# excamera/alfalfa

Measured on AMD Instinct MI355X. Metric: 1080p macroblocks/s decode (bit-exact vs reference), higher is better.
Workload: dtype u8

## Files before the change

### alfalfa_amd/capi.py

```python
import ctypes as C
import os

import numpy as np

from . import build as _build

AA_OK = 0
ERR_NAMES = {-1: "Invalid", -2: "Unsupported", -3: "LogicError", -4: "OutOfRange", -5: "HipError",
             -6: "NoDevice", -7: "BadArgument", -8: "NoMemory"}

AA_MB_HAS_NONZERO, AA_MB_HAS_Y2, AA_MB_INTER, AA_MB_SKIP, AA_MB_LF_SKIP_INNER = 1, 2, 4, 8, 16

MB_INFO_DTYPE = np.dtype([("y_mode", "u1"), ("uv_mode", "u1"), ("ref_frame", "u1"), ("segment_id", "u1"),
                          ("flags", "u1"), ("lf_level", "u1"), ("split_partition", "u1"), ("reserved", "u1"),
                          ("nz_mask", "<u4"), ("coeff_index", "<u4"), ("u", "u1", (64,))])
assert MB_INFO_DTYPE.itemsize == 80


class FrameHeader(C.Structure):
    _fields_ = [(n, C.c_uint8) for n in (
        "key_frame", "show_frame", "loop_filter_level", "sharpness_level", "num_dct_partitions",
        "segmentation_enabled", "filter_adjustments_enabled", "refresh_last", "refresh_golden",
        "refresh_alternate", "copy_buffer_to_golden", "copy_buffer_to_alternate", "sign_bias_golden",
        "sign_bias_alternate", "q_index", "has_intra_mb")] + [
        ("mb_width", C.c_uint16), ("mb_height", C.c_uint16), ("width", C.c_uint16), ("height", C.c_uint16),
        ("quant", (C.c_uint16 * 6) * 4), ("num_macroblocks", C.c_uint32), ("num_coeff_blocks", C.c_uint32),
        ("num_intra_mbs", C.c_uint32), ("compressed_size", C.c_uint32)]

    def as_dict(self):
        d = {n: getattr(self, n) for n, _ in self._fields_ if n != "quant"}
        d["quant"] = [[self.quant[s][k] for k in range(6)] for s in range(4)]
        return d


class FrameIn(C.Structure):
    _fields_ = [("stream", C.c_void_p), ("data", C.c_char_p), ("size", C.c_size_t)]


class KernelStats(C.Structure):
    _fields_ = [("recon_inter_ms", C.c_double), ("recon_intra_ms", C.c_double), ("loopfilter_ms", C.c_double),
                ("recon_inter_launches", C.c_uint64), ("recon_intra_launches", C.c_uint64),
                ("loopfilter_launches", C.c_uint64), ("macroblocks", C.c_uint64),
                ("parse_headers_ms", C.c_double), ("parse_tokens_ms", C.c_double), ("parse_launches", C.c_uint64),
                ("parsed_macroblocks", C.c_uint64), ("recon_split_ms", C.c_double), ("recon_split_launches", C.c_uint64),
                ("pool_waits", C.c_uint64), ("pool_wait_ms", C.c_double), ("parse_wait_ms", C.c_double),
                ("bind_wait_ms", C.c_double), ("alloc_ms", C.c_double), ("slab_mallocs", C.c_uint64),
                ("token_steps", C.c_uint64), ("token_frames", C.c_uint64), ("worker_launches", C.c_uint64), ("worker_wgs", C.c_uint64),
                ("worker_retires", C.c_uint64), ("heap_grows", C.c_uint64), ("heap_mapped_bytes", C.c_uint64), ("nomem_retries", C.c_uint64), ("frames_evicted", C.c_uint64), ("host_routed_frames", C.c_uint64),
                ("row_handoff_stale_polls", C.c_uint64), ("row_handoff_rereads", C.c_uint64), ("packed_frames", C.c_uint64), ("packed_words", C.c_uint64), ("packed_blocks", C.c_uint64),
                ("host_batch_ms", C.c_double), ("host_batch_parse_wall_ms", C.c_double), ("host_batch_parse_cpu_ms", C.c_double), ("host_batch_arena_ms", C.c_double),
                ("pinned_allocs", C.c_uint64)]


class CtxInfo(C.Structure):
    _fields_ = [(n, C.c_uint64) for n in ("memory_limit_bytes", "pool_bytes", "pool_free_bytes", "pool_pending_bytes", "heap_mapped_bytes", "heap_limit_bytes", "heap_used_bytes",
                                          "pinned_host_bytes")] + [
        (n, C.c_uint32) for n in ("heap_is_virtual", "token_lanes_per_workgroup", "token_workgroups_capacity", "token_workgroups_alive",
                                  "token_lane_lds_bytes", "token_workgroup_lds_bytes", "jobs_waiting", "compute_units")] + [
        ("heap_free_chunks", C.c_int32), ("lanes_starved", C.c_uint32), ("token_profile", C.c_uint64 * 8),
        ("packed_coefficients", C.c_uint32), ("lane_per_partition", C.c_uint32), ("clock_mhz", C.c_uint32), ("host_share_ms", C.c_uint32), ("host_rate_kb_per_ms", C.c_uint32), ("reserved1", C.c_uint32), ("stream_concurrency", C.c_uint32), ("streams_needed", C.c_uint32),
        ("host_waited_parse_ms", C.c_uint32), ("host_waited_compute_ms", C.c_uint32)]


AA_RGB_U8_HWC3, AA_RGB_U8_HWC4, AA_RGB_U8_CHW, AA_RGB_F16_CHW, AA_RGB_BF16_CHW, AA_RGB_F32_CHW = range(6)


class RgbTarget(C.Structure):
    _fields_ = [("dst", C.c_void_p), ("row_stride", C.c_int64), ("plane_stride", C.c_int64)]


AA_QUALITY_Y, AA_QUALITY_YUV = 1, 3


class QualityRef(C.Structure):
    _fields_ = [("y", C.c_void_p), ("u", C.c_void_p), ("v", C.c_void_p), ("y_stride", C.c_int64), ("uv_stride", C.c_int64)]


class AlfalfaError(RuntimeError):

    def __init__(self, code, message):
        super().__init__("%s: %s" % (ERR_NAMES.get(code, str(code)), message))
        self.code, self.kind, self.message = code, ERR_NAMES.get(code, str(code)), message


_P = C.c_void_p
_U8P = C.POINTER(C.c_uint8)
SYMBOLS = [
    ("aa_last_error", C.c_char_p, []), ("aa_abi_version", C.c_int, []), ("aa_runtime_prepare", C.c_int, []), ("aa_host_cpus", C.c_int, []), ("aa_device_count", C.c_int, []),
    ("aa_parser_create", C.c_int, [C.c_uint16, C.c_uint16, C.POINTER(_P)]), ("aa_parser_destroy", None, [_P]),
    ("aa_parser_parse", C.c_int, [_P, C.c_char_p, C.c_size_t, C.POINTER(FrameHeader), _P, _P]),
    ("aa_parser_get_probs", C.c_int, [_P, _U8P]), ("aa_parser_set_error_concealment", C.c_int, [_P, C.c_int]),
    ("aa_parse_frame_tag", C.c_int, [C.c_char_p, C.c_size_t, C.c_uint16, C.c_uint16, C.c_int] + [C.POINTER(C.c_int)] * 4),
    ("aa_stream_set_error_concealment", C.c_int, [_P, C.c_int]), ("aa_stream_error_concealment", C.c_int, [_P]),
    ("aa_parser_get_segmentation", C.c_int, [_P, C.POINTER(C.c_int), C.POINTER(C.c_int), C.POINTER(C.c_int8), C.POINTER(C.c_int8), _U8P]),
    ("aa_parser_get_filter_adjustments", C.c_int, [_P, C.POINTER(C.c_int), C.POINTER(C.c_int8), C.POINTER(C.c_int8)]),
    ("aa_parser_serialize_state", C.c_int, [_P, _P, C.c_size_t, _P]), ("aa_parser_deserialize_state", C.c_int, [_P, _P, C.c_size_t]),
    ("aa_stream_serialize", C.c_int, [_P, _P, C.c_size_t, _P]), ("aa_stream_deserialize", C.c_int, [_P, _P, C.c_size_t]),
    ("aa_parser_state_size", C.c_size_t, [_P]), ("aa_parser_export_state", C.c_int, [_P, _P, C.c_size_t]),
    ("aa_parser_import_state", C.c_int, [_P, C.c_char_p, C.c_size_t]),
    ("aa_stream_state_size", C.c_size_t, [_P]), ("aa_stream_export_state", C.c_int, [_P, _P, C.c_size_t]),
    ("aa_stream_import_state", C.c_int, [_P, C.c_char_p, C.c_size_t]),
    ("aa_stream_export_raster", C.c_int, [_P, C.c_int, _P, _P, _P]),
    ("aa_ctx_create", C.c_int, [C.c_int, C.POINTER(_P)]), ("aa_ctx_destroy", None, [_P]), ("aa_ctx_sync", C.c_int, [_P]),
    ("aa_ctx_memory", C.c_int, [_P, C.POINTER(C.c_size_t), C.POINTER(C.c_size_t)]),
    ("aa_ctx_set_memory_limit", C.c_int, [_P, C.c_size_t]), ("aa_ctx_set_packed_coefficients", C.c_int, [_P, C.c_int]), ("aa_ctx_set_host_share_ms", C.c_int, [_P, C.c_double]), ("aa_ctx_set_lane_per_partition", C.c_int, [_P, C.c_int]), ("aa_ctx_get_info", C.c_int, [_P, C.POINTER(CtxInfo)]),
    ("aa_ctx_set_schedule", C.c_int, [_P, C.c_int]), ("aa_ctx_clear_error", C.c_int, [_P]), ("aa_ctx_compute_stream", _P, [_P]), ("aa_ctx_copy_stream", _P, [_P]),
    ("aa_stream_create", C.c_int, [_P, C.c_uint16, C.c_uint16, C.POINTER(_P)]), ("aa_stream_destroy", None, [_P]),
    ("aa_stream_parse", C.c_int, [_P, C.c_char_p, C.c_size_t, C.POINTER(C.c_int), C.POINTER(FrameHeader)]),
    ("aa_stream_append_records", C.c_int, [_P, C.POINTER(FrameHeader), _P, _P, C.POINTER(C.c_int)]),
    ("aa_stream_upload", C.c_int, [_P]), ("aa_stream_release_staging", C.c_int, [_P]),
    ("aa_decode_batch", C.c_int, [_P, C.POINTER(_P), C.c_int, C.POINTER(C.c_int)]),
    ("aa_stream_decode", C.c_int, [_P, C.c_char_p, C.c_size_t, C.POINTER(C.c_int), C.POINTER(C.c_int)]),
    ("aa_submit_frames", C.c_int, [_P, C.POINTER(FrameIn), C.c_int, C.POINTER(C.c_int), C.c_int]),
    ("aa_submit_frames_ex", C.c_int, [_P, C.POINTER(FrameIn), C.c_int, C.POINTER(C.c_int), C.c_int, C.c_uint]),
    ("aa_launch_tokens", C.c_int, [_P, C.c_int, C.POINTER(C.c_int)]),
    ("aa_ssim_host", C.c_int, [C.c_char_p, C.c_char_p, C.c_int, C.c_int, C.POINTER(C.c_double)]),
    ("aa_stream_lf_search", C.c_int, [_P, C.c_char_p, C.c_size_t, C.c_void_p, C.c_int, C.c_int, C.POINTER(C.c_int), C.POINTER(C.c_double),
                                      C.POINTER(C.c_double), C.c_void_p]),
    ("aa_stream_frame_header", C.c_int, [_P, C.c_int, C.POINTER(FrameHeader)]),
    ("aa_stream_read_records", C.c_int, [_P, C.c_int, _P, _P, C.c_size_t]),
    ("aa_stream_frame_count", C.c_int, [_P]), ("aa_stream_release_before", C.c_int, [_P, C.c_int]),
    ("aa_stream_rewind", C.c_int, [_P]), ("aa_stream_rewind_to", C.c_int, [_P, C.c_int]),
    ("aa_stream_download", C.c_int, [_P, C.c_int, _P, _P, _P]),
    ("aa_pinned_alloc", C.c_int, [_P, C.c_size_t, C.POINTER(_P)]), ("aa_pinned_free", None, [_P]),
    ("aa_stream_download_async", C.c_int, [_P, C.c_int, _P, _P, _P]), ("aa_stream_download_wait", C.c_int, [_P]),
    ("aa_download_batch_async", C.c_int, [_P, C.POINTER(_P), C.c_int, C.POINTER(C.c_int), _P, C.c_size_t]), ("aa_ctx_download_wait", C.c_int, [_P]), ("aa_ctx_download_wait_until", C.c_int, [_P, C.c_int]),
    ("aa_stream_raster_device", C.c_int, [_P, C.c_int, C.POINTER(_P), C.POINTER(_P), C.POINTER(_P)]),
    ("aa_render_rgb_async", C.c_int, [_P, C.POINTER(_P), C.c_int, C.POINTER(C.c_int), C.c_int, C.POINTER(RgbTarget),
                                      C.POINTER(C.c_double), C.POINTER(C.c_double), _P]),
    ("aa_quality_batch_async", C.c_int, [_P, C.POINTER(_P), C.c_int, C.POINTER(C.c_int), C.POINTER(QualityRef), C.c_int, _P, _P, _P]),
    ("aa_stream_references", C.c_int, [_P, C.POINTER(C.c_int), C.POINTER(C.c_int), C.POINTER(C.c_int)]),
    ("aa_stream_reference_slots", C.c_int, [_P, C.POINTER(C.c_int)]),
    ("aa_stream_import_reference", C.c_int, [_P, _P, _P, _P]),
    ("aa_stream_import_reference_host", C.c_int, [_P, _P, _P, _P]),
# ... 54 lines not shown
```

### alfalfa_amd/csrc/device_types.h

```cpp
#pragma once
#include <stdint.h>

#include "../../include/alfalfa_amd.h"

struct aa_dev_frame {
  uint8_t * cur[3];
  const uint8_t * ref[4][3];
  const aa_mb_info * mbs;
  const int16_t * coeffs;
  const unsigned long long * intra_rows;
  uint16_t quant[4][6];
  uint16_t mbw, mbh;
  uint8_t key_frame;
  uint8_t loop_filter_level;
  uint8_t sharpness;
  uint8_t has_intra;
  uint32_t packed;
};

struct aa_raster_binding {
  aa_dev_frame * job;
  uint8_t * cur[3];
  const uint8_t * ref[3][3];
};

struct aa_gather_job {
  const uint8_t * src;
  size_t bytes;
};

struct aa_rgb_job {
  const uint8_t * plane[3];
  uint8_t * dst;
  int64_t row_stride, plane_stride;
  uint32_t stride_y, stride_c;
  uint32_t width, height;
  uint32_t groups;
  uint32_t pad;
};

#define AA_QUALITY_STRIP_ROWS 8
#define AA_QUALITY_CHUNK_WINDOWS 480
struct aa_quality_job {
  const uint8_t * a, * b;
  int64_t stride_a, stride_b;
  uint32_t w4, h4;
  uint32_t groups;
  uint32_t strips, chunks;
  uint32_t pad;
  uint64_t out_off;
};

#define AA_MAX_XCD 16

#define AA_SYNC_WS_DUMP 140
#define AA_SYNC_WS_RESCUES 132
struct aa_sync_ws {
  int error;
  int where[3];
  int dump[AA_SYNC_WS_DUMP];
  int ticket[AA_MAX_XCD];
  int progress[1];
};
#define AA_SYNC_WS_ZERO_FROM ( 16 + 4 * AA_SYNC_WS_DUMP )

#define AA_MAX_BATCH 480

struct aa_frame_list {
  const aa_dev_frame * f[AA_MAX_BATCH];
};

struct aa_seg_stream { uint8_t * map; uint32_t first, count; };

#define AA_MAX_WORKER_GRIDS 16
struct aa_tok_mirror {
  uint32_t seq;
  uint32_t q_head, q_publish, q_reserve;
  int32_t pool_avail;
  uint32_t pool_starving;
  uint32_t exited[AA_MAX_WORKER_GRIDS];
  unsigned long long prof[8];
};

namespace aa {
struct ParseJob;
struct TokQueue; struct CoeffPool; struct Heap;
int launch_parse_mb_headers( const ParseJob * jobs, const uint32_t * order, int n, void * stream );
int launch_segment_fixup( const ParseJob * jobs, const aa_seg_stream * streams, int n_streams, const uint32_t * order, void * stream );
void token_worker_shape( uint32_t lane_bytes, int n_cus, int * lanes_out, uint32_t * lds_out, int * wgs_per_cu_out );
int launch_token_workers( TokQueue * q, unsigned long long * slots, const Heap & heap, uint32_t * exited, const uint32_t * retire, uint32_t gen, uint32_t spread,
                          unsigned long long * prof, unsigned long long linger_ticks, int wgs, int lanes, uint32_t lane_bytes, uint32_t lds, bool packed, uint32_t mp_hint, void * stream,
                          uint32_t * cu_slots = nullptr, uint32_t cu_cap = 0 );
#define AA_CU_SLOTS ( 16 * 256 )
int launch_enqueue_jobs( TokQueue * q, unsigned long long * slots, const ParseJob * jobs, const uint32_t * order, int n, void * stream );
int launch_pool_push_range( const Heap & heap, uint32_t first, uint32_t count, void * stream );
int launch_pool_free_lists( const Heap & heap, const uint32_t * const * lists, int n, void * stream );
int launch_mirror_counters( const TokQueue * q, const CoeffPool * pool, const uint32_t * exited, int n_grids, const unsigned long long * prof, aa_tok_mirror * out, uint32_t seq, void * stream );
int launch_recon_inter4( const aa_frame_list & list, int n, unsigned max_mbs, void * stream );
int launch_recon_inter( const aa_frame_list & list, int n, unsigned max_mbs, bool split_only, void * stream );
int launch_recon_intra_diagonal( const aa_frame_list & list, int n, int diagonal, int row_lo, int rows, void * stream );
int launch_loopfilter_diagonal( const aa_frame_list & list, int n, int diagonal, int row_lo, int rows, void * stream );
int launch_recon_intra4( const aa_frame_list & list, int n_groups, int mbh_max, aa_sync_ws * ws, int n_xcd, void * stream );
int launch_loopfilter_rows4( const aa_frame_list & list, int n_groups, int mbh_max, int mbw_max, aa_sync_ws * ws, uint8_t * boundary, int n_xcd, void * stream );
int launch_probe_xcds( int * out16, int blocks, void * stream );
int launch_probe_concurrency( uint32_t * counter, uint32_t * seen, uint32_t n, unsigned long long timeout_ticks, int slot, void * stream );
int launch_bind_rasters( const aa_raster_binding * b, int n, void * stream );
int launch_gather_rasters( const aa_gather_job * jobs, int n, uint8_t * staging, size_t stride, size_t max_bytes, void * stream );
int launch_render_rgb( const aa_rgb_job * jobs, int n, int format, const uint32_t * table, uint32_t max_threads, void * stream );
int launch_lf_relevel( const aa_mb_info * src, aa_mb_info * dst, unsigned nmb, uint32_t levels, void * stream );
int launch_ssim_windows( const uint8_t * a, const uint8_t * b, int width, int height, float * out, void * stream );
int launch_quality( const aa_quality_job * jobs, int n_planes, uint32_t max_blocks, float * group_values, double * ssim, unsigned long long * sse, void * stream );
}
```

### alfalfa_amd/csrc/parse_kernels.hip

```cpp
#include <hip/hip_runtime.h>

#include <algorithm>

#include "device_types.h"
#include "tok_fsm.hh"
#include "coeff_pack.hh"

#ifndef AA_WORKER_PRIO
#define AA_WORKER_PRIO 3
#endif

namespace {

using aa::ParseJob;

__global__ __launch_bounds__( 64 ) void k_parse_mb_headers( const ParseJob * jobs, const uint32_t * order, int n, int lanes )
{
  __builtin_amdgcn_s_setprio( 2 );

  __shared__ aa::HeaderTables s_tables;
  __shared__ aa::HeaderParams s_params[16];
  const int lane = threadIdx.x;
  for ( uint32_t k = lane; k < sizeof( aa::HeaderTables ) / 4; k += 64 ) reinterpret_cast<uint32_t *>( &s_tables )[k] = reinterpret_cast<const uint32_t *>( &aa::kHeaderTables )[k];
  const int slot = blockIdx.x * lanes + lane;
  const bool mine = lane < lanes && lane < 16 && slot < n;
  const ParseJob * Jp = mine ? &jobs[order[slot]] : nullptr;
  if ( Jp ) {
    const uint32_t * src = reinterpret_cast<const uint32_t *>( static_cast<const aa::HeaderParams *>( &Jp->fp ) );
    for ( uint32_t k = 0; k < sizeof( aa::HeaderParams ) / 4; k++ ) reinterpret_cast<uint32_t *>( &s_params[lane] )[k] = src[k];
  }
  __syncthreads();
  if ( !Jp ) return;
  const ParseJob & J = *Jp;
  if ( J.nmb == 0 ) return;
  const aa::HeaderParams & fp = s_params[lane];
  const aa::HeaderTables & T = s_tables;
  aa::BoolReader32 bd;
  aa::BoolState st; st.bitpos = fp.bd_bitpos; st.range = fp.bd_range; st.active = fp.bd_active;
  bd.resume( J.data + fp.first_off, fp.first_size, st );
  const unsigned mbw = fp.mbw, mbh = fp.mbh;
  const unsigned words_per_row = ( mbw + 63 ) / 64;
  uint32_t intra = 0, split = 0;
  unsigned mi = 0;
  const uint32_t mp_stride = J.mp_stride, mp_base = J.flags_padded, nparts = fp.nparts;
  for ( unsigned row = 0; row < mbh; row++ ) {
    unsigned long long word = 0;
    const uint32_t mp_row = mp_stride ? mp_base + ( row % nparts ) * mp_stride + ( row / nparts ) * mbw : 0u;
    for ( unsigned col = 0; col < mbw; col++, mi++ ) {
      const uint8_t flags = aa::parse_mb_header( bd, fp, T, J.mbs, mi, col, row, static_cast<uint8_t *>( nullptr ) );
      J.mbflags[mi] = flags;
      if ( mp_stride ) J.mbflags[mp_row + col] = flags;
      if ( !( flags & AA_MB_INTER ) ) { intra++; word |= 1ull << ( col & 63 ); }
      else if ( J.mbs[mi].y_mode == aa::SPLITMV ) split = 1;
      if ( ( col & 63 ) == 63 || col + 1 == mbw ) { J.intra_rows[row * words_per_row + ( col >> 6 )] = word; word = 0; }
    }
  }
  J.summary->num_intra_mbs = intra;
  J.summary->has_split = split;
}

__global__ __launch_bounds__( 256 ) void k_segment_fixup( const ParseJob * jobs, const aa_seg_stream * streams, const uint32_t * order )
{
  const aa_seg_stream s = streams[blockIdx.x];
  for ( uint32_t k = 0; k < s.count; k++ ) {
    const uint32_t o = order[s.first + k];
    const ParseJob & J = jobs[o & 0x7FFFFFFFu];
    if ( !J.fp.seg_enabled || J.nmb == 0 ) continue;
    if ( o >> 31 ) {
      for ( uint32_t mi = threadIdx.x; mi < J.nmb; mi += blockDim.x ) s.map[mi] = 3;
      __syncthreads();
    }
    for ( uint32_t mi = threadIdx.x; mi < J.nmb; mi += blockDim.x ) aa::segment_fixup( J.fp, J.mbs[mi], s.map[mi] );
    __syncthreads();
  }
}

struct WorkerArgs {
  aa::TokQueue * q;
  unsigned long long * slots;
  aa::Heap heap;
  uint32_t * exited;
  const uint32_t * retire;
  uint32_t gen;
  uint32_t spread;
  unsigned long long * prof;
  unsigned long long linger_ticks;
  int lanes;
  uint32_t lane_bytes;
  uint32_t mp_hint;
  uint32_t * cu_slots;
  uint32_t cu_cap;
  int16_t * sink;
};

__device__ inline uint32_t queue_take( aa::TokQueue * q, uint32_t want, uint32_t spread, uint32_t * base )
{
  uint32_t h = AA_AT_LOAD( &q->head );
  for ( uint32_t tries = 0; ; tries++ ) {
    const uint32_t avail = AA_AT_LOAD( &q->publish ) - h;
    if ( static_cast<int32_t>( avail ) <= 0 ) return 0;
    const uint32_t share = ( avail + spread - 1u ) / spread;
    const uint32_t n = want < share ? want : share;
    uint32_t expect = h;
    if ( __hip_atomic_compare_exchange_strong( &q->head, &expect, h + n, __ATOMIC_RELAXED, __ATOMIC_RELAXED, __HIP_MEMORY_SCOPE_AGENT ) ) { *base = h; return n; }
    h = expect;
    const uint32_t r = ( blockIdx.x * 2654435761u + tries * 40503u ) >> 27;
    for ( uint32_t k = 0; k <= ( r & ( tries < 4 ? 3u : tries < 8 ? 15u : 31u ) ); k++ ) __builtin_amdgcn_s_sleep( 16 );
    if ( tries > 2048 ) h = AA_AT_LOAD( &q->head );
  }
}

__device__ inline int nth_set_bit( unsigned long long mask, uint32_t n )
{
  for ( uint32_t k = 0; k < n; k++ ) mask &= mask - 1ull;
  return __ffsll( static_cast<long long>( mask ) ) - 1;
}

template <bool PK, bool MP>
__global__ __launch_bounds__( 64 ) void k_token_workers( const WorkerArgs a )
{
  extern __shared__ __attribute__( ( aligned( 16 ) ) ) uint8_t smem[];
  const int lane = threadIdx.x;
#if AA_WORKER_PRIO
  __builtin_amdgcn_s_setprio( AA_WORKER_PRIO );
#endif
  uint32_t cu_slot = 0;
  if ( a.cu_slots ) {
    const uint32_t hw = __builtin_amdgcn_s_getreg( 4 | ( 8 << 6 ) | ( 7 << 11 ) ), xcc = __builtin_amdgcn_s_getreg( 20 | ( 0 << 6 ) | ( 3 << 11 ) );
    cu_slot = ( ( xcc & 15u ) << 8 ) | ( hw & 255u );
    uint32_t before = 0;
    if ( lane == 0 ) before = AA_AT_ADD( &a.cu_slots[cu_slot], 1u );
    before = __shfl( before, 0 );
    if ( before >= a.cu_cap ) {
      if ( lane == 0 ) { AA_AT_ADD( &a.cu_slots[cu_slot], 0xFFFFFFFFu ); AA_AT_ADD( &a.cu_slots[AA_CU_SLOTS - 1], 1u ); AA_AT_ADD( a.exited, 1u ); }
      return;
    }
  }
  for ( uint32_t k = lane; k < aa::tok::kTablesBytes / 4; k += 64 ) reinterpret_cast<uint32_t *>( smem )[k] = aa::tok::table_word( k );
  __syncthreads();
  aa::tok::Lane L;
  aa::tok::Frame F {};
// ... 79 lines not shown
      }
      backoff = 0;
      continue;
    }
    idle_since = 0;
    const unsigned long long t_b = profiling ? wall_clock64() : 0ull;
    if ( active ) aa::tok::top_up<MP>( L, smem, F );
    const unsigned long long t_c = profiling ? wall_clock64() : 0ull;
    aa::tok::run_period<PK, MP>( L, smem, F, a.heap, profiling, pp );
    if ( profiling ) {
      const unsigned long long t_d = wall_clock64();
      p_look += t_b - t_a; p_topup += t_c - t_b; p_period += t_d - t_c;
      p_lanes += static_cast<unsigned long long>( __popcll( __ballot( active ) ) ); p_periods++;
      if ( ( p_periods & 1023ull ) == 0 ) {
        if ( lane == 0 ) prof_flush();
        pp = { 0, 0, 0 }; p_look = p_topup = p_period = p_lanes = p_periods = 0;
      }
    }
  }
  if ( lane == 0 ) {
    if ( profiling ) prof_flush();
    if ( a.cu_slots ) AA_AT_ADD( &a.cu_slots[cu_slot], 0xFFFFFFFFu );
    AA_AT_ADD( a.exited, 1u );
  }
}

__global__ __launch_bounds__( 64 ) void k_enqueue_jobs( aa::TokQueue * q, unsigned long long * slots, const ParseJob * jobs, const uint32_t * order, int n )
{
  __shared__ uint32_t s_base;
  if ( threadIdx.x == 0 ) s_base = AA_AT_ADD( &q->reserve, static_cast<uint32_t>( n ) );
  __syncthreads();
  const uint32_t base = s_base, mask = q->mask;
  for ( int i = threadIdx.x; i < n; i += 64 ) AA_AT_STORE( &slots[( base + i ) & mask], reinterpret_cast<unsigned long long>( &jobs[order[i]] ) );
  __syncthreads();
  if ( threadIdx.x == 0 ) {
    __builtin_amdgcn_fence( __ATOMIC_RELEASE, "agent" );
    asm volatile( "s_waitcnt vmcnt(0)" ::: "memory" );
    while ( AA_AT_LOAD( &q->publish ) != base ) __builtin_amdgcn_s_sleep( 8 );
    AA_AT_STORE( &q->publish, base + static_cast<uint32_t>( n ) );
  }
}

__device__ inline void pool_push_wave( const aa::Heap & H, const AA_GLOBAL uint32_t * ids, uint32_t first, uint32_t n_mine )
{
  __shared__ uint32_t s_off[65];
  __shared__ uint32_t s_pbase;
  s_off[threadIdx.x + 1] = n_mine;
  __syncthreads();
  if ( threadIdx.x == 0 ) {
    s_off[0] = 0;
    for ( int i = 1; i <= 64; i++ ) s_off[i] += s_off[i - 1];
    s_pbase = s_off[64] ? AA_AT_ADD( &H.pool->reserve, s_off[64] ) : 0u;
  }
  __syncthreads();
  const uint32_t b = s_pbase + s_off[threadIdx.x], mask = H.pool->mask, total = s_off[64];
  for ( uint32_t i = 0; i < n_mine; i++ ) AA_AT_STORE( &H.ring[( b + i ) & mask], ids ? ids[i] : first + i );
  __syncthreads();
  if ( threadIdx.x == 0 && total ) {
    __builtin_amdgcn_fence( __ATOMIC_RELEASE, "agent" );
    asm volatile( "s_waitcnt vmcnt(0)" ::: "memory" );
    while ( AA_AT_LOAD( &H.pool->publish ) != s_pbase ) __builtin_amdgcn_s_sleep( 8 );
    AA_AT_STORE( &H.pool->publish, s_pbase + total );
    AA_AT_ADD_REL( &H.pool->avail, static_cast<int32_t>( total ) );
  }
}
__global__ __launch_bounds__( 64 ) void k_pool_push_range( aa::Heap heap, uint32_t first, uint32_t count )
{
  const uint32_t per = ( count + 63u ) / 64u, lo = threadIdx.x * per;
  const uint32_t mine = lo >= count ? 0u : ( count - lo < per ? count - lo : per );
  pool_push_wave( heap, nullptr, first + lo, mine );
}
struct FreeLists { const uint32_t * l[AA_MAX_BATCH]; };
__global__ __launch_bounds__( 64 ) void k_pool_free_lists( aa::Heap heap, const FreeLists lists, int n )
{
  const int i = blockIdx.x * 64 + threadIdx.x;
  const AA_GLOBAL uint32_t * l = ( i < n && lists.l[i] ) ? (const AA_GLOBAL uint32_t *) lists.l[i] : nullptr;
  pool_push_wave( heap, l ? l + 1 : nullptr, 0, l ? l[0] : 0u );
}
__global__ void k_mirror_counters( const aa::TokQueue * q, const aa::CoeffPool * pool, const uint32_t * exited, int n_grids, const unsigned long long * prof, aa_tok_mirror * out, uint32_t seq )
{
  if ( threadIdx.x || blockIdx.x ) return;
  if ( prof ) for ( int k = 0; k < 8; k++ ) out->prof[k] = AA_AT_LOAD( &prof[k] );
  out->q_head = AA_AT_LOAD( &q->head ); out->q_publish = AA_AT_LOAD( &q->publish ); out->q_reserve = AA_AT_LOAD( &q->reserve );
  if ( pool ) { out->pool_avail = AA_AT_LOAD( &pool->avail ); out->pool_starving = AA_AT_LOAD( &pool->starving ); }
  for ( int g = 0; g < n_grids; g++ ) out->exited[g] = AA_AT_LOAD( &exited[g] );
  __builtin_amdgcn_fence( __ATOMIC_RELEASE, "" );
  asm volatile( "s_waitcnt vmcnt(0)" ::: "memory" );
  __hip_atomic_store( &out->seq, seq, __ATOMIC_RELAXED, __HIP_MEMORY_SCOPE_SYSTEM );
}

}

namespace aa {

static int parse_lanes_env()
{
  static const int lanes = [] {
    const char * e = getenv( "ALFALFA_AMD_PARSE_LANES" );
    const int v = e ? atoi( e ) : 0;
    return v < 0 ? 0 : ( v > 64 ? 64 : v );
  }();
  return lanes;
}
static int header_lanes() { const int v = parse_lanes_env(); return v ? std::min( v, 16 ) : 16; }

constexpr uint32_t kLdsPerCu = 160u * 1024u, kLdsGranule = 512u;
static uint32_t env_u32( const char * name, uint32_t dflt ) { const char * e = getenv( name ); return e ? static_cast<uint32_t>( atoi( e ) ) : dflt; }
static const uint32_t kWgsPerCu = std::max( 1u, std::min( 16u, env_u32( "ALFALFA_AMD_WGS_PER_CU", 3u ) ) );
static const uint32_t kMaxLanes = std::max( 1u, std::min( 64u, env_u32( "ALFALFA_AMD_MAX_LANES", 30u ) ) );
struct TokenShape { int lanes; uint32_t lds; int per_cu; };
static TokenShape token_launch_shape( uint32_t lane_bytes )
{
  for ( uint32_t n = kWgsPerCu; n >= 1; n-- ) {
    const uint32_t request = std::min( 65536u, ( kLdsPerCu / ( n + 1 ) / kLdsGranule + 1 ) * kLdsGranule );
    if ( request < tok::kTablesBytes + lane_bytes || request * n > kLdsPerCu ) continue;
    const int lanes = static_cast<int>( std::min<uint32_t>( kMaxLanes, ( request - tok::kTablesBytes ) / lane_bytes ) );
    return { lanes, request, static_cast<int>( n ) };
  }
  return { 0, 0, 0 };
}

int launch_parse_mb_headers( const ParseJob * jobs, const uint32_t * order, int n, void * stream )
{
  const int lanes = header_lanes();
  hipLaunchKernelGGL( k_parse_mb_headers, dim3( ( n + lanes - 1 ) / lanes ), dim3( 64 ), 0, static_cast<hipStream_t>( stream ), jobs, order, n, lanes );
  return static_cast<int>( hipGetLastError() );
}

int launch_segment_fixup( const ParseJob * jobs, const aa_seg_stream * streams, int n_streams, const uint32_t * order, void * stream )
{
  hipLaunchKernelGGL( k_segment_fixup, dim3( n_streams ), dim3( 256 ), 0, static_cast<hipStream_t>( stream ), jobs, streams, order );
  return static_cast<int>( hipGetLastError() );
}

void token_worker_shape( uint32_t lane_bytes, int n_cus, int * lanes_out, uint32_t * lds_out, int * wgs_per_cu_out )
{
  int lanes = parse_lanes_env();
  uint32_t lds = 0;
  if ( lanes ) {
    if ( static_cast<uint32_t>( lanes ) * lane_bytes + tok::kTablesBytes > 65536u ) lanes = static_cast<int>( ( 65536u - tok::kTablesBytes ) / lane_bytes );
    lds = static_cast<uint32_t>( lanes ) * lane_bytes + tok::kTablesBytes;
  } else {
    const TokenShape sh = token_launch_shape( lane_bytes );
    lanes = sh.lanes; lds = sh.lds;
  }
  (void) n_cus;
  static const bool lds_exact = env_u32( "ALFALFA_AMD_LDS_EXACT", 1u ) != 0u;
  static const uint32_t wgs_cap = env_u32( "ALFALFA_AMD_WGS_CAP_PER_CU", lds_exact && !parse_lanes_env() ? kWgsPerCu : 0u );
  if ( lds_exact && lanes > 0 ) lds = ( ( tok::kTablesBytes + static_cast<uint32_t>( lanes ) * lane_bytes + kLdsGranule - 1u ) / kLdsGranule ) * kLdsGranule;
  *lanes_out = lanes; *lds_out = lds;
  int per_cu = lds ? static_cast<int>( kLdsPerCu / lds ) : 0;
  if ( wgs_cap && per_cu > static_cast<int>( wgs_cap ) ) per_cu = static_cast<int>( wgs_cap );
  *wgs_per_cu_out = per_cu;
}

int launch_token_workers( TokQueue * q, unsigned long long * slots, const Heap & heap, uint32_t * exited, const uint32_t * retire, uint32_t gen, uint32_t spread,
                          unsigned long long * prof, unsigned long long linger_ticks, int wgs, int lanes, uint32_t lane_bytes, uint32_t lds, bool packed, uint32_t mp_hint, void * stream,
                          uint32_t * cu_slots, uint32_t cu_cap )
{
  if ( lanes < 1 || wgs < 1 ) return static_cast<int>( hipErrorInvalidValue );
  WorkerArgs a;
  a.q = q; a.slots = slots; a.heap = heap; a.exited = exited; a.retire = retire; a.gen = gen; a.spread = spread ? spread : 1u; a.prof = prof; a.linger_ticks = linger_ticks; a.lanes = lanes; a.lane_bytes = lane_bytes;
  a.mp_hint = mp_hint ? mp_hint : 1u;
  a.cu_slots = cu_cap ? cu_slots : nullptr; a.cu_cap = cu_cap;
  a.sink = reinterpret_cast<int16_t *>( cu_slots + AA_CU_SLOTS / 2 );
  if ( mp_hint ) {
    if ( packed ) hipLaunchKernelGGL( ( k_token_workers<true, true> ), dim3( wgs ), dim3( 64 ), lds, static_cast<hipStream_t>( stream ), a );
    else hipLaunchKernelGGL( ( k_token_workers<false, true> ), dim3( wgs ), dim3( 64 ), lds, static_cast<hipStream_t>( stream ), a );
  } else {
    if ( packed ) hipLaunchKernelGGL( ( k_token_workers<true, false> ), dim3( wgs ), dim3( 64 ), lds, static_cast<hipStream_t>( stream ), a );
    else hipLaunchKernelGGL( ( k_token_workers<false, false> ), dim3( wgs ), dim3( 64 ), lds, static_cast<hipStream_t>( stream ), a );
  }
  return static_cast<int>( hipGetLastError() );
}

int launch_enqueue_jobs( TokQueue * q, unsigned long long * slots, const ParseJob * jobs, const uint32_t * order, int n, void * stream )
{
  hipLaunchKernelGGL( k_enqueue_jobs, dim3( 1 ), dim3( 64 ), 0, static_cast<hipStream_t>( stream ), q, slots, jobs, order, n );
  return static_cast<int>( hipGetLastError() );
}

int launch_pool_push_range( const Heap & heap, uint32_t first, uint32_t count, void * stream )
{
  hipLaunchKernelGGL( k_pool_push_range, dim3( 1 ), dim3( 64 ), 0, static_cast<hipStream_t>( stream ), heap, first, count );
  return static_cast<int>( hipGetLastError() );
}

int launch_pool_free_lists( const Heap & heap, const uint32_t * const * lists, int n, void * stream )
{
  for ( int base = 0; base < n; base += AA_MAX_BATCH ) {
    FreeLists fl;
    const int cnt = std::min( AA_MAX_BATCH, n - base );
    for ( int i = 0; i < AA_MAX_BATCH; i++ ) fl.l[i] = i < cnt ? lists[base + i] : nullptr;
    hipLaunchKernelGGL( k_pool_free_lists, dim3( ( cnt + 63 ) / 64 ), dim3( 64 ), 0, static_cast<hipStream_t>( stream ), heap, fl, cnt );
    if ( hipError_t e = hipGetLastError() ) return static_cast<int>( e );
  }
  return 0;
}

int launch_mirror_counters( const TokQueue * q, const CoeffPool * pool, const uint32_t * exited, int n_grids, const unsigned long long * prof, aa_tok_mirror * out, uint32_t seq, void * stream )
{
  hipLaunchKernelGGL( k_mirror_counters, dim3( 1 ), dim3( 64 ), 0, static_cast<hipStream_t>( stream ), q, pool, exited, n_grids, prof, out, seq );
  return static_cast<int>( hipGetLastError() );
}

}
```

### alfalfa_amd/csrc/runtime_ctx.inc

```

extern "C" {

const char * aa_last_error( void ) { return g_last_error.c_str(); }
int aa_host_cpus( void ) { return effective_cpus(); }
int aa_runtime_prepare( void )
{
  const bool was_set = std::getenv( "GPU_MAX_HW_QUEUES" ) != nullptr;
  setenv( "GPU_MAX_HW_QUEUES", "16", 0 );
  return was_set ? 1 : 0;
}
int aa_abi_version( void ) { return AA_ABI_VERSION; }
int aa_device_count( void ) { int n = 0; if ( hipGetDeviceCount( &n ) != hipSuccess ) return 0; return n; }

void aa_raster_geometry( uint16_t width, uint16_t height, uint32_t * pw, uint32_t * ph )
{
  if ( pw ) *pw = 16u * ( ( width + 15u ) / 16u );
  if ( ph ) *ph = 16u * ( ( height + 15u ) / 16u );
}

aa_status aa_parser_create( uint16_t width, uint16_t height, aa_parser ** out )
{
  if ( !out || !width || !height ) return fail( AA_ERR_ARGUMENT, "aa_parser_create: bad argument" );
  *out = new ( std::nothrow ) aa_parser( width, height );
  return *out ? AA_OK : fail( AA_ERR_ARGUMENT, "out of memory" );
// ... 265 lines not shown
    out->memory_limit_bytes = ctx->pool_soft_limit; out->pool_bytes = ctx->pool_bytes; out->pinned_host_bytes = ctx->pinned_bytes;
    for ( auto & kv : ctx->dev_free ) out->pool_free_bytes += kv.first * kv.second.size();
    for ( auto & pf : ctx->pending_free ) out->pool_pending_bytes += pf.bytes;
    if ( ctx->cur_slab ) out->pool_free_bytes += kSlabBytes - ctx->slab_used;
    out->pool_free_bytes += ctx->compute_free_bytes;
    for ( auto & h : ctx->compute_hold ) out->pool_pending_bytes += h.second;
  }
  out->heap_mapped_bytes = T.heap_mapped; out->heap_limit_bytes = T.heap_va;
  out->heap_used_bytes = static_cast<uint64_t>( std::max<int64_t>( 0, T.chunks_committed ) ) * kChunkBytesHeap;
  out->heap_is_virtual = T.vmm ? 1u : 0u;
  out->packed_coefficients = T.packed ? 1u : 0u;
  out->lane_per_partition = T.lane_per_partition ? 1u : 0u;
  out->token_lanes_per_workgroup = static_cast<uint32_t>( T.lanes ); out->token_workgroups_capacity = static_cast<uint32_t>( T.cap_wgs );
  out->token_lane_lds_bytes = T.lane_bytes; out->token_workgroup_lds_bytes = T.lds;
  out->compute_units = static_cast<uint32_t>( T.n_cus );
  out->host_share_ms = static_cast<uint32_t>( ctx->host_share_ms + 0.5 );
  out->host_rate_kb_per_ms = ctx->host_lanes.parse_us.load() ? static_cast<uint32_t>( host_lanes_rate( ctx ) / 1e3 + 0.5 ) : 0u;
  out->stream_concurrency = ctx->stream_concurrency; out->streams_needed = ctx->streams_needed;
  out->host_waited_parse_ms = static_cast<uint32_t>( ctx->stats.parse_wait_ms ); out->host_waited_compute_ms = static_cast<uint32_t>( ctx->stats.bind_wait_ms );
  if ( !ctx->clock_mhz ) { int khz = 0; if ( hipDeviceGetAttribute( &khz, hipDeviceAttributeClockRate, ctx->device ) == hipSuccess ) ctx->clock_mhz = static_cast<uint32_t>( khz / 1000 ); else (void) hipGetLastError(); }
  out->clock_mhz = ctx->clock_mhz;
  if ( T.ready ) {
    if ( aa_status st = tok_peek_mirror( ctx ) ) return st;
    out->heap_free_chunks = T.mirror_host->pool_avail; out->lanes_starved = T.mirror_host->pool_starving;
    for ( int k = 0; k < 8; k++ ) out->token_profile[k] = T.mirror_host->prof[k];
    uint32_t alive = 0;
    for ( int g = 0; g < aa_ctx::Tok::kSlots; g++ ) alive += T.slot[g].launched - T.mirror_host->exited[g];
    out->token_workgroups_alive = alive;
    const int32_t waiting = static_cast<int32_t>( static_cast<uint32_t>( T.jobs_enqueued ) - T.mirror_host->q_head );
    out->jobs_waiting = waiting > 0 ? static_cast<uint32_t>( waiting ) : 0u;
  }
  return AA_OK;
}
aa_status aa_ctx_set_lane_per_partition( aa_ctx * ctx, int on )
{
  if ( !ctx ) return fail( AA_ERR_ARGUMENT, "null context" );
  if ( ctx->tok.ready && ctx->tok.lane_per_partition != ( on != 0 ) ) return fail( AA_ERR_LOGIC, "aa_ctx_set_lane_per_partition: frames have been submitted to this context already" );
  ctx->tok.lane_per_partition = on != 0;
  return AA_OK;
}
aa_status aa_ctx_set_host_share_ms( aa_ctx * ctx, double ms )
{
  if ( !ctx || !( ms >= 0 ) ) return fail( AA_ERR_ARGUMENT, "aa_ctx_set_host_share_ms: bad argument" );
  ctx->host_share_ms = ms;
  return AA_OK;
}
aa_status aa_ctx_set_packed_coefficients( aa_ctx * ctx, int on )
{
  if ( !ctx ) return fail( AA_ERR_ARGUMENT, "null context" );
  if ( ctx->tok.ready && ctx->tok.packed != ( on != 0 ) ) return fail( AA_ERR_LOGIC, "aa_ctx_set_packed_coefficients: frames have been submitted to this context already" );
  ctx->tok.packed = on != 0;
  return AA_OK;
}
aa_status aa_ctx_clear_error( aa_ctx * ctx )
{
  if ( !ctx ) return fail( AA_ERR_ARGUMENT, "null ctx" );
  if ( aa_status st = set_device( ctx ) ) return st;
  HIP_TRY( hipStreamSynchronize( ctx->compute ) );
  if ( ctx->ws ) { HIP_TRY( hipMemsetAsync( ctx->ws, 0, AA_SYNC_WS_ZERO_FROM, ctx->compute ) ); HIP_TRY( hipStreamSynchronize( ctx->compute ) ); }
  return AA_OK;
}
aa_status aa_ctx_set_schedule( aa_ctx * ctx, int schedule )
{
  if ( !ctx || ( schedule != AA_SCHEDULE_ROWS && schedule != AA_SCHEDULE_DIAGONAL ) ) return fail( AA_ERR_ARGUMENT, "aa_ctx_set_schedule: bad argument" );
  ctx->schedule = schedule;
  return AA_OK;
}
void * aa_ctx_compute_stream( aa_ctx * ctx ) { return ctx ? ctx->compute : nullptr; }
void * aa_ctx_copy_stream( aa_ctx * ctx ) { return ctx ? ctx->copy : nullptr; }
aa_status aa_ctx_profile( aa_ctx * ctx, int enable )
{
  if ( !ctx ) return fail( AA_ERR_ARGUMENT, "null ctx" );
  if ( !enable ) { (void) hipStreamSynchronize( ctx->compute ); for ( auto ps : ctx->parse_streams ) (void) hipStreamSynchronize( ps ); drain_profile( ctx ); }
  ctx->profile = enable != 0;
  return AA_OK;
}
aa_status aa_ctx_kernel_stats( aa_ctx * ctx, aa_kernel_stats * out, int reset )
{
  if ( !ctx || !out ) return fail( AA_ERR_ARGUMENT, "null argument" );
  HIP_TRY( hipStreamSynchronize( ctx->compute ) );
  for ( auto ps : ctx->parse_streams ) HIP_TRY( hipStreamSynchronize( ps ) );
  drain_profile( ctx );
  ctx->stats.heap_mapped_bytes = ctx->tok.heap_mapped;
  if ( ctx->ws ) {
    int rescued[6] = {};
    HIP_TRY( hipMemcpy( rescued, &ctx->ws->dump[AA_SYNC_WS_RESCUES], sizeof rescued, hipMemcpyDeviceToHost ) );
    ctx->stats.row_handoff_rereads = static_cast<uint64_t>( rescued[0] );
    ctx->stats.row_handoff_stale_polls = static_cast<uint64_t>( rescued[3] );
    ctx->row_handoff_by_kernel[0] = rescued[4]; ctx->row_handoff_by_kernel[1] = rescued[5];
    if ( const char * e = std::getenv( "ALFALFA_AMD_HANDOFF_REPORT" ) ) if ( atoi( e ) )
      std::fprintf( stderr, "alfalfa_amd: row hand-off waits ended by the second look: %d (k_recon_intra4 %d, k_loopfilter_rows4 %d); system-scope load saw it %d, L2 read-modify-write %d; poll repeated still stale %d\n",
                    rescued[0], rescued[4], rescued[5], rescued[1], rescued[2], rescued[3] );
  }
  const uint64_t lanes_us = ctx->host_lanes.parse_us.load();
  ctx->stats.host_batch_parse_cpu_ms = static_cast<double>( lanes_us - ctx->host_lanes.parse_us_mark ) / 1e3;
  *out = ctx->stats;
  if ( reset ) { ctx->stats = aa_kernel_stats {}; ctx->host_lanes.parse_us_mark = lanes_us; }
  return AA_OK;
}

aa_status aa_stream_create( aa_ctx * ctx, uint16_t width, uint16_t height, aa_stream ** out )
{
  if ( !ctx || !out || !width || !height ) return fail( AA_ERR_ARGUMENT, "aa_stream_create: bad argument" );
  if ( aa_status st = set_device( ctx ) ) return st;
  std::unique_ptr<aa_stream> s( new aa_stream( ctx, width, height ) );
  aa_raster_geometry( width, height, &s->pw, &s->ph );
  s->plane_bytes[0] = size_t( s->pw ) * s->ph;
  s->plane_bytes[1] = s->plane_bytes[2] = size_t( s->pw / 2 ) * ( s->ph / 2 );
  s->slot_bytes = align_up( s->plane_bytes[0] + 2 * s->plane_bytes[1] );
  uint8_t * blank = nullptr;
  {
    std::lock_guard<std::mutex> g( ctx->blank_mu );
    auto it = ctx->blank.find( s->slot_bytes );
    if ( it != ctx->blank.end() ) blank = it->second;
    else {
      if ( aa_status st = dev_alloc( ctx, s->slot_bytes, &blank ) ) return st;
      hipError_t e = hipMemsetAsync( blank, 0, s->slot_bytes, ctx->compute );
      if ( e == hipSuccess ) e = hipStreamSynchronize( ctx->compute );
      if ( e != hipSuccess ) { dev_free( ctx, blank, s->slot_bytes ); return hip_fail( e, "hipMemsetAsync (blank reference raster)" ); }
      ctx->blank[s->slot_bytes] = blank;
    }
  }
  Slot sl; sl.dev = blank; sl.shared = true;
  s->slots.push_back( sl );
  const int slot = 0;
  for ( int i = 0; i < 3; i++ ) { s->cur_ref_slot[i] = -1; s->cur_ref_frame[i] = -1; }
  for ( int i = 0; i < 3; i++ ) set_ref( s.get(), i, slot, -1 );
  ctx->refs++;
  *out = s.release();
  return AA_OK;
}
void aa_stream_destroy( aa_stream * s )
{
  if ( !s ) return;
  aa_ctx * ctx = s->ctx;
  (void) hipSetDevice( ctx->device );
  bool staged = false;
  for ( auto & c : s->chunks ) if ( c.host && c.uploaded ) staged = true;
  if ( staged ) (void) hipStreamSynchronize( ctx->copy );
  for ( auto & f : s->frames ) if ( f.batch && f.batch->hdr_done && !f.enqueued && !f.records_released ) (void) hipEventSynchronize( f.batch->hdr_done );
  for ( auto & f : s->frames ) release_records( s, f, true );
  for ( auto & c : s->chunks ) {
    if ( c.host ) { std::lock_guard<std::mutex> g( ctx->pool_mu ); ctx->pinned_pool.emplace_back( c.host, c.pinned_bytes ); c.host = nullptr; }
    if ( c.dev ) { dev_free( ctx, c.dev, c.dev_bytes, true ); c.dev = nullptr; }
  }
  for ( auto & sl : s->slots ) if ( sl.dev && !sl.shared ) dev_free_compute( ctx, sl.dev, s->slot_bytes );
  dev_free( ctx, s->dev_segmap, size_t( s->parser.mb_width() ) * s->parser.mb_height(), true );
  delete s;
  if ( --ctx->refs == 0 ) ctx_free( ctx );
}

}
```

### alfalfa_amd/csrc/runtime_decode.inc

```
extern "C" {

static aa_status resolve_summary( aa_stream * s, FrameRec & r )
{
  if ( !r.summary_pending ) return AA_OK;
  aa_ctx * ctx = s->ctx;
  auto & T = ctx->tok;
  Batch * b = r.batch;
  if ( !b || !r.summary ) return fail( AA_ERR_LOGIC, "frame records were released before the frame was decoded" );
  if ( b->tokens_pending ) if ( aa_status st = launch_tokens_of( ctx, b ) ) return st;
  volatile aa::FrameSummary * sum = r.summary;
  for ( int attempt = 0; ; attempt++ ) {
    if ( aa_status st = tok_wait_done( ctx, sum ) ) return st;
    if ( sum->status != aa::TOK_NO_MEMORY ) break;
    ctx->stats.nomem_retries++;
    const uint32_t worst = aa::chunk_list_entries( r.hdr.num_macroblocks, T.lane_per_partition ? 8u : 1u );
    {
      std::lock_guard<std::mutex> g( ctx->pool_mu );
      if ( !r.chunks_returned ) { T.pending_lists.push_back( r.chunk_list ); r.chunks_returned = true; T.chunks_committed -= r.est_chunks; r.est_chunks = 0; }
      flush_chunk_frees( ctx );
      if ( !T.pending_lists.empty() ) return fail( AA_ERR_HIP, "k_pool_free_lists could not be launched" );
    }
    HIP_TRY( hipStreamSynchronize( ctx->compute ) );
    if ( aa_status st = tok_grow_heap( ctx, T.heap_mapped + static_cast<size_t>( worst ) * kChunkBytesHeap ) ) return st;
    if ( aa_status st = tok_refresh_mirror( ctx ) ) return st;
    if ( T.mirror_host->pool_avail < static_cast<int32_t>( worst ) ) {
      if ( aa_status st = tok_quiesce( ctx ) ) return st;
      if ( aa_status st = tok_refresh_mirror( ctx ) ) return st;
    }
    if ( T.mirror_host->pool_avail < static_cast<int32_t>( worst ) ) {
      int32_t have = T.mirror_host->pool_avail;
      std::lock_guard<std::mutex> g( ctx->pool_mu );
      for ( auto bi = T.batches.rbegin(); bi != T.batches.rend() && have < static_cast<int32_t>( worst ); ++bi ) {
        Batch * vb = *bi;
        volatile aa::FrameSummary * sums = reinterpret_cast<volatile aa::FrameSummary *>( vb->host + vb->summaries_off );
        for ( int i = vb->n - 1; i >= 0 && have < static_cast<int32_t>( worst ); i-- ) {
          if ( !vb->items[i].live ) continue;
          aa_stream * vs = vb->items[i].s;
          FrameRec & v = vs->frames[vb->items[i].frame];
          if ( &v == &r || vb->items[i].on_host || !v.enqueued || v.records_released || v.chunks_returned || !sums[i].done || vb->items[i].frame < vs->next_submit ) continue;
          T.pending_lists.push_back( v.chunk_list );
          have += static_cast<int32_t>( sums[i].num_chunks );
          v.chunks_returned = true; v.summary_pending = true;
          T.chunks_committed -= v.est_chunks; v.est_chunks = 0;
          sums[i].status = aa::TOK_NO_MEMORY;
          ctx->stats.frames_evicted++;
        }
      }
      flush_chunk_frees( ctx );
      if ( !T.pending_lists.empty() ) return fail( AA_ERR_HIP, "k_pool_free_lists could not be launched" );
    }
    HIP_TRY( hipStreamSynchronize( ctx->compute ) );
    if ( aa_status st = tok_refresh_mirror( ctx ) ) return st;
    if ( attempt >= 8 || T.mirror_host->pool_avail < static_cast<int32_t>( worst ) )
      return fail( AA_ERR_NO_MEMORY, "device parser: the coefficient heap is exhausted (" + std::to_string( T.heap_mapped >> 20 ) + " MiB mapped, "
                                     + std::to_string( T.mirror_host->pool_avail ) + " chunks free, this frame may need " + std::to_string( worst )
                                     + "): release decoded frames (aa_stream_release_before) or raise the limit (aa_ctx_set_memory_limit); the call can be repeated" );
    sum->status = 0; sum->done = 0; sum->num_chunks = 0;
    r.chunks_returned = false;
    r.est_chunks = worst; T.chunks_committed += worst;
    __atomic_thread_fence( __ATOMIC_SEQ_CST );
    if ( int e = aa::launch_enqueue_jobs( T.q, T.slots, r.parse_job, T.one_dev, 1, T.util ) ) return hip_fail( static_cast<hipError_t>( e ), "k_enqueue_jobs" );
    T.jobs_enqueued += 1;
    if ( std::find( T.inflight.begin(), T.inflight.end(), b ) == T.inflight.end() ) T.inflight.push_back( b );
    if ( aa_status st = tok_service( ctx ) ) return st;
  }
  if ( sum->status == aa::TOK_HOST_FAILED ) return fail( AA_ERR_HIP, "host lane: the frame's records could not be placed in device memory" );
  if ( sum->status == aa::TOK_STEP_BOUND ) return fail( AA_ERR_HIP, "device parser: a token lane exceeded the step bound of its frame size (records are not valid)" );
  r.hdr.num_coeff_blocks = sum->num_coeff_blocks;
  r.hdr.num_intra_mbs = sum->num_intra_mbs;
  r.hdr.has_intra_mb = sum->num_intra_mbs != 0;
  r.has_split = sum->has_split != 0;
  r.intra_diagonals.assign( r.hdr.mb_width + 2 * ( r.hdr.mb_height - 1 ), r.hdr.has_intra_mb ? 1 : 0 );
  T.chunks_committed += static_cast<int64_t>( sum->num_chunks ) - static_cast<int64_t>( r.est_chunks );
  r.est_chunks = sum->num_chunks;
  if ( r.hdr.compressed_size ) T.blocks_per_byte += 0.05 * ( static_cast<double>( sum->num_coeff_blocks ) / r.hdr.compressed_size - T.blocks_per_byte );
  if ( r.hdr.compressed_size && r.packed_pos ) T.words_per_byte += 0.05 * ( static_cast<double>( sum->packed_words ) / r.hdr.compressed_size - T.words_per_byte );
  if ( r.packed_pos ) { ctx->stats.packed_frames++; ctx->stats.packed_words += sum->packed_words; ctx->stats.packed_blocks += sum->num_coeff_blocks; }
  ctx->stats.token_steps += sum->steps; ctx->stats.token_frames++;
  r.summary_pending = false;
  return AA_OK;
}

aa_status aa_stream_frame_header( aa_stream * s, int fi, aa_frame_header * out )
{
  if ( !s || !out || fi < 0 || fi >= static_cast<int>( s->frames.size() ) ) return fail( AA_ERR_ARGUMENT, "aa_stream_frame_header: bad argument" );
  if ( aa_status st = set_device( s->ctx ) ) return st;
  if ( aa_status st = resolve_summary( s, s->frames[fi] ) ) return st;
  *out = s->frames[fi].hdr;
  return AA_OK;
}

aa_status aa_stream_read_records( aa_stream * s, int fi, aa_mb_info * mb_out, int16_t * coeff_out, size_t coeff_capacity_blocks )
{
  if ( !s || fi < 0 || fi >= static_cast<int>( s->frames.size() ) ) return fail( AA_ERR_ARGUMENT, "aa_stream_read_records: bad argument" );
  if ( aa_status st = set_device( s->ctx ) ) return st;
  FrameRec & r = s->frames[fi];
  if ( r.records_released ) return fail( AA_ERR_LOGIC, "aa_stream_read_records: frame records were released" );
  if ( aa_status st = resolve_summary( s, r ) ) return st;
  if ( aa_status st = aa_stream_upload( s ) ) return st;
  HIP_TRY( hipStreamSynchronize( s->ctx->copy ) );
  aa_dev_frame job;
  HIP_TRY( hipMemcpy( &job, r.dev_job, sizeof job, hipMemcpyDeviceToHost ) );
  if ( coeff_out && coeff_capacity_blocks < r.hdr.num_coeff_blocks ) return fail( AA_ERR_ARGUMENT, "aa_stream_read_records: coefficient buffer too small" );
  if ( !r.chunk_list ) {
    if ( mb_out ) HIP_TRY( hipMemcpy( mb_out, job.mbs, size_t( r.hdr.num_macroblocks ) * sizeof( aa_mb_info ), hipMemcpyDeviceToHost ) );
    if ( coeff_out ) HIP_TRY( hipMemcpy( coeff_out, job.coeffs, size_t( r.hdr.num_coeff_blocks ) * 32, hipMemcpyDeviceToHost ) );
    return AA_OK;
  }
  std::vector<aa_mb_info> mbs( r.hdr.num_macroblocks );
  HIP_TRY( hipMemcpy( mbs.data(), job.mbs, mbs.size() * sizeof( aa_mb_info ), hipMemcpyDeviceToHost ) );
  std::vector<uint32_t> list( size_t( r.est_chunks ) + 1 );
  HIP_TRY( hipMemcpy( list.data(), r.chunk_list, list.size() * sizeof( uint32_t ), hipMemcpyDeviceToHost ) );
  if ( list[0] != r.est_chunks ) return fail( AA_ERR_LOGIC, "aa_stream_read_records: chunk list disagrees with the parse summary" );
  if ( r.packed_pos ) {
    std::vector<uint32_t> pos( r.hdr.num_macroblocks );
    HIP_TRY( hipMemcpy( pos.data(), r.packed_pos, pos.size() * sizeof( uint32_t ), hipMemcpyDeviceToHost ) );
    std::vector<std::vector<int16_t>> words( list[0] );
    if ( coeff_out )
      for ( uint32_t k = 0; k < list[0]; k++ ) {
        words[k].resize( aa::kChunkWords );
        HIP_TRY( hipMemcpy( words[k].data(), s->ctx->tok.heap + size_t( list[1 + k] ) * kChunkBytesHeap, kChunkBytesHeap, hipMemcpyDeviceToHost ) );
      }
    uint32_t running = 0;
    for ( size_t mi = 0; mi < mbs.size(); mi++ ) {
      aa_mb_info & mb = mbs[mi];
      const uint32_t nblk = aa::pack::blocks_of( mb.nz_mask );
      if ( nblk && coeff_out ) {
        const uint32_t ord = pos[mi] >> 15, off = pos[mi] & ( aa::kChunkWords - 1u );
        if ( ord >= list[0] || running + nblk > r.hdr.num_coeff_blocks )
          return fail( AA_ERR_LOGIC, "aa_stream_read_records: a macroblock's coefficients lie outside the frame's chunks" );
        const int16_t * w = words[ord].data() + off, * end = words[ord].data() + aa::kChunkWords;
        if ( w + aa::pack::kMaskSlots > end ) return fail( AA_ERR_LOGIC, "aa_stream_read_records: packed coefficients run past their chunk" );
        uint32_t values = 0;
        for ( uint32_t b = 0; b < 25; b++ ) if ( ( mb.nz_mask >> b ) & 1u ) values += aa::pack::popc( static_cast<uint16_t>( w[b] ) );
        if ( w + aa::pack::kMaskSlots + values > end ) return fail( AA_ERR_LOGIC, "aa_stream_read_records: packed coefficients run past their chunk" );
        if ( ( static_cast<unsigned long long>( mb.reserved ) << 32 | mb.coeff_index ) != static_cast<unsigned long long>( list[1 + ord] ) * aa::kChunkWords + off )
          return fail( AA_ERR_LOGIC, "aa_stream_read_records: a macroblock's word offset disagrees with its place in the frame's chunks" );
        aa::pack::expand_macroblock( w, mb.nz_mask, coeff_out + size_t( running ) * 16 );
      }
      mb.coeff_index = running; mb.reserved = 0;
      running += nblk;
    }
    if ( running != r.hdr.num_coeff_blocks ) return fail( AA_ERR_LOGIC, "aa_stream_read_records: non-zero masks disagree with the parse summary" );
    if ( mb_out ) std::memcpy( mb_out, mbs.data(), mbs.size() * sizeof( aa_mb_info ) );
    return AA_OK;
  }
  std::map<uint32_t, std::vector<uint8_t>> chunk;
  if ( coeff_out )
    for ( uint32_t k = 0; k < list[0]; k++ ) {
// ... 263 lines not shown
```

### alfalfa_amd/csrc/runtime_records.inc

```

static uint8_t * slot_plane( aa_stream * s, int slot, int plane )
{
  uint8_t * p = s->slots[slot].dev;
  if ( plane >= 1 ) p += s->plane_bytes[0];
  if ( plane >= 2 ) p += s->plane_bytes[1];
  return p;
}

namespace {

void release_records( aa_stream * s, FrameRec & f, bool deferred )
{
  if ( f.records_released ) return;
  aa_ctx * ctx = s->ctx;
  bool parsed = false;
  if ( f.enqueued && f.summary ) parsed = tok_wait_done( ctx, f.summary ) == AA_OK;
  if ( !parsed && f.enqueued && f.summary && f.batch && f.batch_item >= 0 && f.batch_item < static_cast<int>( f.batch->items.size() ) && f.batch->items[f.batch_item].on_host ) {
    while ( !summary_done( f.summary ) ) usleep( 200 );
  }
  f.records_released = true;
  if ( f.rec_block ) {
    const bool has_chunks = parsed && f.chunk_list && !f.chunks_returned;
    if ( has_chunks ) { std::lock_guard<std::mutex> g( ctx->pool_mu ); ctx->tok.pending_lists.push_back( f.chunk_list ); ctx->open_epoch_used = true; f.chunks_returned = true; }
    if ( !f.rec_in_arena ) dev_free( ctx, f.rec_block, f.rec_bytes, deferred || has_chunks );
    f.rec_block = nullptr; f.chunk_list = nullptr; f.packed_pos = nullptr;
    ctx->tok.chunks_committed -= f.est_chunks; f.est_chunks = 0;
  }
  if ( Batch * b = f.batch ) {
    if ( f.batch_item >= 0 && f.batch_item < static_cast<int>( b->items.size() ) ) {
      Batch::Item & bi = b->items[f.batch_item];
      if ( bi.host_dense ) { dev_free( ctx, bi.host_dense, bi.host_dense_bytes, true ); bi.host_dense = nullptr; }
    }
    bool last;
    { std::lock_guard<std::mutex> g( ctx->pool_mu ); last = --b->live == 0; }
    if ( f.batch_item >= 0 && f.batch_item < static_cast<int>( b->items.size() ) ) b->items[f.batch_item].live = false;
    if ( last ) {
      if ( b->tokens_pending ) ctx->deferred.erase( std::remove( ctx->deferred.begin(), ctx->deferred.end(), b ), ctx->deferred.end() );
      ctx->tok.inflight.erase( std::remove( ctx->tok.inflight.begin(), ctx->tok.inflight.end(), b ), ctx->tok.inflight.end() );
      ctx->tok.batches.erase( std::remove( ctx->tok.batches.begin(), ctx->tok.batches.end(), b ), ctx->tok.batches.end() );
      if ( b->hdr_done ) { (void) hipEventSynchronize( b->hdr_done ); (void) hipEventDestroy( b->hdr_done ); }
      { std::lock_guard<std::mutex> g( ctx->pool_mu ); ctx->pinned_pool.emplace_back( b->host, b->host_bytes ); }
      dev_free( ctx, b->dev, b->dev_bytes, true );
      delete b;
    }
    f.batch = nullptr; f.summary = nullptr; f.parse_job = nullptr;
  }
  if ( f.chunk >= 0 && f.chunk < static_cast<int>( s->chunks.size() ) ) {
    Chunk & c = s->chunks[f.chunk];
    const bool is_tail = f.chunk + 1 == static_cast<int>( s->chunks.size() ) && c.host != nullptr;
    if ( --c.live_frames == 0 && !is_tail && c.dev ) {
      if ( c.host ) { std::lock_guard<std::mutex> g( ctx->pool_mu ); ctx->pinned_pool.emplace_back( c.host, c.pinned_bytes ); c.host = nullptr; }
      dev_free( ctx, c.dev, c.dev_bytes, deferred ); c.dev = nullptr;
    }
  }
  f.host_job = nullptr; f.dev_job = nullptr;
}

uint8_t * pinned_get( aa_ctx * ctx, size_t bytes, size_t * got )
{
  {
    std::lock_guard<std::mutex> g( ctx->pool_mu );
    auto & pool = ctx->pinned_pool;
    for ( size_t i = 0; i < pool.size(); i++ )
      if ( pool[i].second >= bytes && pool[i].second <= bytes + bytes / 2 ) {
        uint8_t * p = pool[i].first; *got = pool[i].second;
        pool[i] = pool.back(); pool.pop_back();
        return p;
      }
  }
  uint8_t * p = nullptr;
  if ( hipHostMalloc( reinterpret_cast<void **>( &p ), bytes, hipHostMallocDefault ) != hipSuccess ) return nullptr;
  *got = bytes;
  { std::lock_guard<std::mutex> g( ctx->pool_mu ); ctx->pinned_bytes += bytes; ctx->stats.pinned_allocs++; }
  return p;
}

void fill_job( const FrameRec & rec, aa_dev_frame * job )
{
  const aa_frame_header & h = rec.hdr;
  std::memset( job, 0, sizeof *job );
  std::memcpy( job->quant, h.quant, sizeof job->quant );
  job->mbw = h.mb_width; job->mbh = h.mb_height;
  job->key_frame = h.key_frame; job->loop_filter_level = h.loop_filter_level;
  job->sharpness = h.sharpness_level; job->has_intra = h.has_intra_mb;
}

aa_status bind_frame( aa_stream * s, int fi, aa_raster_binding * out )
{
  FrameRec & rec = s->frames[fi];
  const aa_frame_header & h = rec.hdr;
  int out_slot;
  if ( aa_status st = alloc_slot( s, &out_slot ) ) return st;
  retain( s, out_slot );
  rec.out_slot = out_slot;
  out->job = const_cast<aa_dev_frame *>( rec.dev_job );
  for ( int p = 0; p < 3; p++ ) out->cur[p] = slot_plane( s, out_slot, p );
  for ( int r = 0; r < 3; r++ ) for ( int p = 0; p < 3; p++ ) out->ref[r][p] = slot_plane( s, s->cur_ref_slot[r], p );
  enum { LAST = 0, GOLDEN = 1, ALT = 2 };
  if ( h.key_frame ) { for ( int i = 0; i < 3; i++ ) set_ref( s, i, out_slot, fi ); }
  else {
    if ( h.copy_buffer_to_alternate == 1 ) set_ref( s, ALT, s->cur_ref_slot[LAST], s->cur_ref_frame[LAST] );
    else if ( h.copy_buffer_to_alternate == 2 ) set_ref( s, ALT, s->cur_ref_slot[GOLDEN], s->cur_ref_frame[GOLDEN] );
    if ( h.copy_buffer_to_golden == 1 ) set_ref( s, GOLDEN, s->cur_ref_slot[LAST], s->cur_ref_frame[LAST] );
    else if ( h.copy_buffer_to_golden == 2 ) set_ref( s, GOLDEN, s->cur_ref_slot[ALT], s->cur_ref_frame[ALT] );
    if ( h.refresh_golden ) set_ref( s, GOLDEN, out_slot, fi );
    if ( h.refresh_alternate ) set_ref( s, ALT, out_slot, fi );
    if ( h.refresh_last ) set_ref( s, LAST, out_slot, fi );
  }
  for ( int i = 0; i < 3; i++ ) rec.ref_after[i] = s->cur_ref_frame[i];
  rec.placed = true;
  if ( !rec.handle_held ) release( s, out_slot );
  return AA_OK;
}

aa_status bind_batch( aa_ctx * ctx, aa_stream * const * streams, int n, const int * frame_index )
{
  int need = 0;
  for ( int i = 0; i < n; i++ ) if ( !streams[i]->frames[frame_index[i]].placed ) need++;
  if ( !need ) return AA_OK;
  aa_ctx::BindBuf & bb = ctx->bind_bufs[ctx->next_bind_buf];
  ctx->next_bind_buf = ( ctx->next_bind_buf + 1 ) % aa_ctx::kBindBufs;
  if ( bb.busy ) {
    const auto t0 = std::chrono::steady_clock::now();
// ... 37 lines not shown
```

### alfalfa_amd/csrc/runtime_submit.inc

```
namespace {
template <class Fill>
aa_status append_host_frame( aa_stream * s, int * frame_index, aa_frame_header * hdr_out, Fill && fill )
{
  if ( aa_status st = set_device( s->ctx ) ) return st;
  const size_t nmb = size_t( s->parser.mb_width() ) * s->parser.mb_height();
  const size_t job_bytes = align_up( sizeof( aa_dev_frame ) );
  const size_t mb_bytes = align_up( nmb * sizeof( aa_mb_info ) );
  const size_t words_per_row = ( s->parser.mb_width() + 63 ) / 64;
  const size_t rows_bytes = align_up( words_per_row * s->parser.mb_height() * sizeof( unsigned long long ) );
  const size_t worst = job_bytes + mb_bytes + rows_bytes + align_up( nmb * 25 * 32 );
  Chunk * c;
  if ( aa_status st = reserve( s, worst, &c ) ) return st;
  const size_t off = c->used;
  aa_dev_frame * job = reinterpret_cast<aa_dev_frame *>( c->host + off );
  aa_mb_info * mbs = reinterpret_cast<aa_mb_info *>( c->host + off + job_bytes );
  unsigned long long * intra_rows = reinterpret_cast<unsigned long long *>( c->host + off + job_bytes + mb_bytes );
  int16_t * coeffs = reinterpret_cast<int16_t *>( c->host + off + job_bytes + mb_bytes + rows_bytes );

  FrameRec rec;
  try { fill( rec.hdr, mbs, coeffs ); }
  catch ( const aa::ParseError & e ) { return fail( e.code, e.message ); }
  const aa_frame_header & h = rec.hdr;
  c->used = off + job_bytes + mb_bytes + rows_bytes + align_up( size_t( h.num_coeff_blocks ) * 32 );

// ... 55 lines not shown
  }
  return append_host_frame( s, frame_index, nullptr, [&]( aa_frame_header & h, aa_mb_info * mbs, int16_t * coeffs ) {
    h = *hdr;
    h.num_intra_mbs = intra; h.has_intra_mb = intra != 0;
    std::memcpy( mbs, mbs_in, nmb * sizeof( aa_mb_info ) );
    if ( hdr->num_coeff_blocks ) std::memcpy( coeffs, coeffs_in, size_t( hdr->num_coeff_blocks ) * 32 );
  } );
}

aa_status aa_stream_upload( aa_stream * s )
{
  if ( !s ) return fail( AA_ERR_ARGUMENT, "null stream" );
  if ( aa_status st = set_device( s->ctx ) ) return st;
  bool any = false;
  for ( auto & c : s->chunks ) {
    if ( c.host && c.uploaded < c.used ) {
      HIP_TRY( hipMemcpyAsync( c.dev + c.uploaded, c.host + c.uploaded, c.used - c.uploaded, hipMemcpyHostToDevice, s->ctx->copy ) );
      c.uploaded = c.used; any = true;
    }
  }
  if ( any ) {
    HIP_TRY( hipEventRecord( s->ctx->upload_done, s->ctx->copy ) );
    HIP_TRY( hipStreamWaitEvent( s->ctx->compute, s->ctx->upload_done, 0 ) );
  }
  return AA_OK;
}

aa_status aa_stream_release_staging( aa_stream * s )
{
  if ( !s ) return fail( AA_ERR_ARGUMENT, "null stream" );
  if ( aa_status st = set_device( s->ctx ) ) return st;
  if ( aa_status st = aa_stream_upload( s ) ) return st;
  HIP_TRY( hipStreamSynchronize( s->ctx->copy ) );
  for ( auto & c : s->chunks ) {
    if ( !c.host ) continue;
    { std::lock_guard<std::mutex> g( s->ctx->pool_mu ); s->ctx->pinned_pool.emplace_back( c.host, c.pinned_bytes ); }
    c.host = nullptr;
    c.capacity = c.used;
  }
  for ( auto & f : s->frames ) f.host_job = nullptr;
  return AA_OK;
}


namespace {
struct SubmitItem {
  aa_stream * s; const uint8_t * data; size_t size;
  size_t data_off;
  size_t rec_off = 0;
  aa_status status = AA_OK; std::string error;
  int frame_index = -1;
  bool seg_enabled = false, seg_reset = false;
  bool on_host = false;
};

aa_status submit_one( Batch * b, SubmitItem & it, int item, aa::ParseJob * jobs_host, aa_dev_frame * dframes_host, bool want_host_lane )
{
  aa_stream * s = it.s;
  aa_ctx * ctx = s->ctx;
  aa::ParseJob & J = jobs_host[item];
  FrameRec rec;
  try { s->parser.parse_header( it.data, it.size, rec.hdr, J.fp ); }
  catch ( const aa::ParseError & e ) { it.error = e.message; return e.code; }
  it.seg_enabled = J.fp.seg_enabled; it.seg_reset = s->parser.segment_map_reset();
  std::memcpy( b->host + it.data_off, it.data, it.size );

  const uint32_t nmb = uint32_t( J.fp.mbw ) * J.fp.mbh;
  const size_t mb_bytes = align_up( size_t( nmb ) * sizeof( aa_mb_info ) );
  const size_t words_per_row = ( J.fp.mbw + 63 ) / 64;
  const size_t rows_bytes = align_up( words_per_row * J.fp.mbh * sizeof( unsigned long long ) );
  const uint32_t flags_padded = ( nmb + 15u ) & ~15u;
  const bool mp = ctx->tok.lane_per_partition && J.fp.nparts > 1;
  const uint32_t mp_stride = mp ? aa::mp_flag_stride( J.fp.mbw, J.fp.mbh, J.fp.nparts ) : 0u;
  const size_t flags_bytes = align_up( size_t( flags_padded ) + size_t( J.fp.nparts ) * mp_stride );
  const size_t list_bytes = align_up( size_t( aa::chunk_list_entries( nmb, mp ? J.fp.nparts : 1u ) ) * sizeof( uint32_t ) );

  const size_t pos_bytes = ctx->tok.packed ? align_up( size_t( nmb ) * sizeof( uint32_t ) ) : 0;
  rec.rec_bytes = mb_bytes + rows_bytes + flags_bytes + list_bytes + pos_bytes;
  rec.rec_block = b->dev + it.rec_off; rec.rec_in_arena = true;
  uint8_t * blk = rec.rec_block;

  J.data = b->dev + it.data_off;
  J.size = static_cast<uint32_t>( it.size ); J.data_padded = ( J.size + 15u ) & ~15u;
  J.nmb = nmb; J.flags_padded = flags_padded; J.mp_stride = mp_stride; J.mp_pad = 0;
  J.mbs = reinterpret_cast<aa_mb_info *>( blk );
  J.intra_rows = reinterpret_cast<unsigned long long *>( blk + mb_bytes );
  J.mbflags = blk + mb_bytes + rows_bytes;
  J.chunk_list = reinterpret_cast<uint32_t *>( blk + mb_bytes + rows_bytes + flags_bytes );
  J.packed_pos = pos_bytes ? reinterpret_cast<uint32_t *>( blk + mb_bytes + rows_bytes + flags_bytes + list_bytes ) : nullptr;
  rec.packed_pos = J.packed_pos; rec.dev_mbs = J.mbs;
  J.summary = reinterpret_cast<aa::FrameSummary *>( b->host_dev + b->summaries_off ) + item;
  rec.chunk_list = J.chunk_list;
  rec.summary = reinterpret_cast<volatile aa::FrameSummary *>( b->host + b->summaries_off ) + item;
  rec.parse_job = reinterpret_cast<const aa::ParseJob *>( b->dev ) + item;

  aa_dev_frame * job = &dframes_host[item];
  rec.hdr.has_intra_mb = 1;
  fill_job( rec, job );
  job->mbs = J.mbs; job->intra_rows = J.intra_rows;
  job->coeffs = reinterpret_cast<const int16_t *>( ctx->tok.heap );
  job->packed = ctx->tok.packed ? 1u : 0u;
  rec.host_job = job;
  rec.dev_job = reinterpret_cast<const aa_dev_frame *>( b->dev + ( reinterpret_cast<uint8_t *>( job ) - b->host ) );
  rec.batch = b; rec.batch_item = item; rec.summary_pending = true;
  if ( want_host_lane && !J.fp.seg_enabled ) {
    it.on_host = true;
    job->packed = 0;
    rec.packed_pos = nullptr; rec.chunk_list = nullptr;
    rec.enqueued = true;
  }
  it.frame_index = static_cast<int>( s->frames.size() );
  s->frames.push_back( std::move( rec ) );
  return AA_OK;
}
}

namespace {
aa_status launch_tokens_of( aa_ctx * ctx, Batch * b )
{
  if ( !b->tokens_pending ) return AA_OK;
  auto & T = ctx->tok;
  aa::ParseJob * jobs_host = reinterpret_cast<aa::ParseJob *>( b->host );
  if ( static_cast<uint32_t>( T.jobs_enqueued ) - T.mirror_host->q_head + static_cast<uint32_t>( b->n ) + 4096u > T.q_slots ) {
    if ( aa_status st = tok_refresh_mirror( ctx ) ) return st;
    if ( static_cast<uint32_t>( T.jobs_enqueued ) - T.mirror_host->q_head + static_cast<uint32_t>( b->n ) + 4096u > T.q_slots )
      if ( aa_status st = tok_quiesce( ctx ) ) return st;
  }
  b->tokens_pending = false;
  ctx->deferred.erase( std::remove( ctx->deferred.begin(), ctx->deferred.end(), b ), ctx->deferred.end() );
  bool dropped = false;
  tok_prune_inflight( ctx );
  for ( int i = 0; i < b->n; i++ ) {
    Batch::Item & it = b->items[i];
    if ( !it.live ) { if ( jobs_host[i].nmb ) { jobs_host[i].nmb = 0; dropped = true; } continue; }
    FrameRec & r = it.s->frames[it.frame];
    if ( it.on_host ) continue;
    r.enqueued = true;
    if ( T.packed ) {
      const double words = std::min( double( aa::kMbWords ) * jobs_host[i].nmb, T.words_per_byte * 1.15 * jobs_host[i].size );
      r.est_chunks = static_cast<uint32_t>( words / ( aa::kChunkWords - aa::kMbWords ) ) + 1u;
    } else {
      const double blocks = std::min( 25.0 * jobs_host[i].nmb, T.blocks_per_byte * 1.15 * jobs_host[i].size );
      r.est_chunks = static_cast<uint32_t>( blocks / ( aa::kChunkBlocks - aa::kMbBlocks ) ) + 1u;
    }
    if ( T.lane_per_partition && jobs_host[i].mp_stride && jobs_host[i].fp.nparts > 1 ) r.est_chunks += static_cast<uint32_t>( jobs_host[i].fp.nparts ) - 1u;
    T.chunks_committed += r.est_chunks;
    ctx->stats.parsed_macroblocks += jobs_host[i].nmb;
  }
  if ( std::find( T.inflight.begin(), T.inflight.end(), b ) == T.inflight.end() ) T.inflight.push_back( b );
  if ( std::find( T.batches.begin(), T.batches.end(), b ) == T.batches.end() ) T.batches.push_back( b );
  if ( aa_status st = tok_grow_heap( ctx, static_cast<size_t>( std::max<int64_t>( 0, T.chunks_committed ) ) * kChunkBytesHeap ) ) return st;
  hipStream_t ps = b->ps;
  if ( b->patch_jobs && dropped ) HIP_TRY( hipMemcpyAsync( b->dev, b->host, b->head_bytes, hipMemcpyHostToDevice, ps ) );
  if ( dropped ) {
    int keep = 0;
    for ( int k = 0; k < b->n_order; k++ ) if ( b->items[b->launch_order_host[k]].live ) b->launch_order_host[keep++] = b->launch_order_host[k];
    b->n_order = keep;
    if ( keep ) HIP_TRY( hipMemcpyAsync( const_cast<uint32_t *>( b->launch_order_dev ), b->launch_order_host, size_t( keep ) * sizeof( uint32_t ), hipMemcpyHostToDevice, ps ) );
  }
  if ( b->n_order > 0 ) {
    if ( int e = aa::launch_enqueue_jobs( T.q, T.slots, reinterpret_cast<const aa::ParseJob *>( b->dev ), b->launch_order_dev, b->n_order, ps ) )
      return hip_fail( static_cast<hipError_t>( e ), "k_enqueue_jobs" );
    T.jobs_enqueued += static_cast<uint64_t>( b->n_order );
  }
  HIP_TRY( hipEventRecord( b->hdr_done, ps ) );
  HIP_TRY( hipEventRecord( ctx->parse_idle[b->parse_stream_index], ps ) );
  return tok_service( ctx, b->hdr_done );
}
}

namespace {
struct HostLaneScratch {
  uint8_t * pin = nullptr; size_t pin_bytes = 0;
  std::vector<uint8_t> above; hipEvent_t ev = nullptr;
  bool fit( size_t bytes )
  {
    if ( bytes <= pin_bytes ) return true;
    if ( pin ) (void) hipHostFree( pin );
    pin = nullptr; pin_bytes = 0;
    if ( hipHostMalloc( reinterpret_cast<void **>( &pin ), bytes, hipHostMallocDefault ) != hipSuccess ) { (void) hipGetLastError(); pin = nullptr; return false; }
    pin_bytes = bytes;
    return true;
  }
};
void host_lane_run( aa_ctx * ctx, Batch * b, int item, HostLaneScratch & S )
{
  const aa::ParseJob & J = reinterpret_cast<const aa::ParseJob *>( b->host )[item];
  volatile aa::FrameSummary * sum = reinterpret_cast<volatile aa::FrameSummary *>( b->host + b->summaries_off ) + item;
  Batch::Item & it = b->items[item];
  const uint32_t mbw = J.fp.mbw, mbh = J.fp.mbh, nmb = mbw * mbh;
  const size_t words_per_row = ( mbw + 63 ) / 64;
  uint32_t status = aa::TOK_OK, blocks = 0, intra = 0, split = 0;
  hipStream_t up = ctx->tok.host_up;
  if ( !S.ev ) status = aa::TOK_HOST_FAILED;
  const size_t mbs_bytes = align_up( size_t( nmb ) * sizeof( aa_mb_info ) ), rows_bytes = align_up( words_per_row * mbh * sizeof( unsigned long long ) );
  try { S.above.resize( size_t( mbw ) * 9 ); } catch ( const std::bad_alloc & ) { status = aa::TOK_HOST_FAILED; }
  if ( status == aa::TOK_OK && !S.fit( mbs_bytes + rows_bytes + size_t( nmb ) * 25 * 32 + 256 ) ) status = aa::TOK_HOST_FAILED;
  if ( status == aa::TOK_OK ) {
    aa_mb_info * mbs = reinterpret_cast<aa_mb_info *>( S.pin );
    unsigned long long * rows = reinterpret_cast<unsigned long long *>( S.pin + mbs_bytes );
    int16_t * coeffs = reinterpret_cast<int16_t *>( S.pin + mbs_bytes + rows_bytes );
    std::memset( static_cast<void *>( mbs ), 0, size_t( nmb ) * sizeof( aa_mb_info ) );
    const double t_parse = now_ms();
    aa::parse_frame_body( b->host + it.data_off, J.fp, mbs, coeffs, S.above.data(), &blocks, &intra );
    ctx->host_lanes.parse_us += static_cast<uint64_t>( ( now_ms() - t_parse ) * 1e3 ); ctx->host_lanes.parsed_bytes += J.size;
    std::memset( rows, 0, words_per_row * mbh * sizeof( unsigned long long ) );
    for ( uint32_t r = 0; r < mbh; r++ ) for ( uint32_t c = 0; c < mbw; c++ ) {
      const aa_mb_info & mb = mbs[r * mbw + c];
      if ( !( mb.flags & AA_MB_INTER ) ) rows[r * words_per_row + ( c >> 6 )] |= 1ull << ( c & 63 );
      else if ( mb.y_mode == aa::SPLITMV ) split = 1;
    }
    uint8_t * dense = nullptr;
    const size_t dense_bytes = align_up( std::max<size_t>( size_t( blocks ) * 32, 32 ) );
    hipError_t e = hipSuccess;
    if ( dev_alloc( ctx, dense_bytes, &dense ) != AA_OK ) status = aa::TOK_HOST_FAILED;
    else {
      it.host_dense = dense; it.host_dense_bytes = dense_bytes;
      e = hipMemcpyAsync( J.mbs, mbs, size_t( nmb ) * sizeof( aa_mb_info ), hipMemcpyHostToDevice, up );
      if ( e == hipSuccess ) e = hipMemcpyAsync( J.intra_rows, rows, words_per_row * mbh * sizeof( unsigned long long ), hipMemcpyHostToDevice, up );
      if ( e == hipSuccess && blocks ) e = hipMemcpyAsync( dense, coeffs, size_t( blocks ) * 32, hipMemcpyHostToDevice, up );
      if ( e == hipSuccess ) {
        uint8_t * job_dev = b->dev + align_up( size_t( b->n ) * sizeof( aa::ParseJob ) ) + size_t( item ) * sizeof( aa_dev_frame );
        const int16_t ** dense_ptr = reinterpret_cast<const int16_t **>( S.pin + S.pin_bytes - 16 );
        *dense_ptr = reinterpret_cast<const int16_t *>( dense );
        e = hipMemcpyAsync( job_dev + offsetof( aa_dev_frame, coeffs ), dense_ptr, sizeof *dense_ptr, hipMemcpyHostToDevice, up );
      }
      if ( e == hipSuccess ) e = hipEventRecord( S.ev, up );
      if ( e == hipSuccess ) e = hipEventSynchronize( S.ev );
      if ( e != hipSuccess ) status = aa::TOK_HOST_FAILED;
    }
  }
  sum->num_coeff_blocks = blocks; sum->num_intra_mbs = intra; sum->has_split = split; sum->steps = 0; sum->num_chunks = 0; sum->packed_words = 0;
  sum->status = status;
  ctx->host_lanes.backlog_bytes -= J.size;
  __atomic_thread_fence( __ATOMIC_RELEASE );
  sum->done = 1u;
}
void host_lanes_main( aa_ctx * ctx )
{
  (void) hipSetDevice( ctx->device );
  HostLaneScratch S;
  for ( int tries = 0; tries < 3 && !S.ev; tries++ )
    if ( hipEventCreateWithFlags( &S.ev, hipEventDisableTiming ) != hipSuccess ) { (void) hipGetLastError(); S.ev = nullptr; usleep( 1000 ); }
  auto & H = ctx->host_lanes;
  for ( ;; ) {
    aa_ctx::HostLanes::Task t;
    {
      std::unique_lock<std::mutex> g( H.mu );
      H.cv.wait( g, [&] { return H.stop || !H.q.empty(); } );
      if ( H.q.empty() ) break;
// ... 191 lines not shown
        }
      }
    };
    if ( nt == 1 ) work();
    else {
      std::vector<std::thread> pool;
      for ( int t = 0; t < nt; t++ ) pool.emplace_back( work );
      for ( auto & t : pool ) t.join();
    }
  }
  aa_status first_error = AA_OK; std::string first_message;
  int appended = 0, max_mbw = 0, max_nparts = 1;
  for ( int i = 0; i < n; i++ ) {
    if ( frame_index_out ) frame_index_out[i] = items[i].frame_index;
    if ( items[i].status == AA_OK ) { appended++; max_mbw = std::max<int>( max_mbw, jobs_host[i].fp.mbw ); max_nparts = std::max<int>( max_nparts, jobs_host[i].fp.nparts ); }
    else {
      jobs_host[i].nmb = 0;
      if ( first_error == AA_OK ) { first_error = items[i].status; first_message = items[i].error; }
    }
  }
  if ( !appended ) {
    { std::lock_guard<std::mutex> g( ctx->pool_mu ); ctx->pinned_pool.emplace_back( b->host, b->host_bytes ); }
    dev_free( ctx, b->dev, b->dev_bytes );
    return fail( first_error, first_message );
  }
  b->live = appended;
  b->items.resize( n );
  for ( int i = 0; i < n; i++ ) { b->items[i] = { items[i].s, items[i].frame_index, items[i].status == AA_OK }; b->items[i].on_host = items[i].status == AA_OK && items[i].on_host; b->items[i].data_off = items[i].data_off; }
  b->head_bytes = jobs_bytes + dframes_bytes;
  b->max_mbw = max_mbw; b->max_nparts = max_nparts;
  if ( ctx->tok.lane_per_partition ) ctx->tok.mp_hint = std::max<uint32_t>( ctx->tok.mp_hint, static_cast<uint32_t>( max_nparts ) );
  struct Abandon {
    aa_ctx * ctx; Batch * b; bool armed = true;
    ~Abandon() {
      if ( !armed ) return;
      const std::string keep = g_last_error;
      {
        volatile aa::FrameSummary * sums = reinterpret_cast<volatile aa::FrameSummary *>( b->host + b->summaries_off );
        for ( size_t i = 0; i < b->items.size(); i++ ) if ( b->items[i].on_host ) { sums[i].status = aa::TOK_HOST_FAILED; sums[i].done = 1u; }
      }
      std::vector<Batch::Item> its = b->items;
      for ( auto & it : its ) if ( it.live ) release_records( it.s, it.s->frames[it.frame], true );
      g_last_error = keep;
    }
  } abandon { ctx, b.release() };
  Batch * const raw = abandon.b;
  if ( aa_status st = tok_set_lane_bytes( ctx, aa::tok::lane_lds_bytes( static_cast<uint32_t>( max_mbw ), max_nparts > 1, ctx->tok.lane_per_partition ) ) ) return st;

  aa_seg_stream * seg_streams = reinterpret_cast<aa_seg_stream *>( raw->host + jobs_bytes + dframes_bytes + sums_bytes );
  uint32_t * seg_order = reinterpret_cast<uint32_t *>( seg_streams + n );
  int n_seg_streams = 0; uint32_t n_seg_order = 0;
  int pick = ctx->next_parse_stream;
  for ( int k = 0; k < ctx->n_parse_streams; k++ ) {
    const int c = ( ctx->next_parse_stream + k ) % ctx->n_parse_streams;
    if ( hipEventQuery( ctx->parse_idle[c] ) == hipSuccess ) { pick = c; break; }
  }
  (void) hipGetLastError();
  ctx->next_parse_stream = ( pick + 1 ) % ctx->n_parse_streams;
  raw->parse_stream_index = pick;
  hipStream_t ps = ctx->parse_streams[pick];
  for ( aa_stream * s : stream_order ) {
    bool any = false;
    for ( int i : by_stream[s] ) if ( items[i].status == AA_OK && items[i].seg_enabled ) any = true;
    if ( !any && !s->segmap_on_device ) continue;
    if ( !any ) continue;
    const size_t map_bytes = size_t( s->parser.mb_width() ) * s->parser.mb_height();
    if ( !s->dev_segmap ) if ( aa_status st = dev_alloc( ctx, map_bytes, &s->dev_segmap ) ) return st;
    if ( !s->segmap_on_device ) {
      HIP_TRY( hipMemcpyAsync( s->dev_segmap, s->parser.segment_map().data(), map_bytes, hipMemcpyHostToDevice, ps ) );
      HIP_TRY( hipStreamSynchronize( ps ) );
      s->segmap_on_device = true;
    }
    aa_seg_stream & ss = seg_streams[n_seg_streams++];
    ss.map = s->dev_segmap; ss.first = n_seg_order; ss.count = 0;
    for ( int i : by_stream[s] ) if ( items[i].status == AA_OK ) { seg_order[n_seg_order++] = static_cast<uint32_t>( i ) | ( items[i].seg_reset ? 0x80000000u : 0u ); ss.count++; }
  }

  uint32_t * launch_order = seg_order + n;
  int n_order = 0;
  for ( int i = 0; i < n; i++ ) if ( items[i].status == AA_OK && !items[i].on_host ) launch_order[n_order++] = static_cast<uint32_t>( i );
  std::stable_sort( launch_order, launch_order + n_order, [&]( uint32_t a, uint32_t b ) { return items[a].size > items[b].size; } );
  const uint32_t * launch_order_dev = reinterpret_cast<const uint32_t *>( raw->dev + ( reinterpret_cast<uint8_t *>( launch_order ) - raw->host ) );

  HIP_TRY( hipEventCreateWithFlags( &raw->hdr_done, hipEventDisableTiming ) );
  HIP_TRY( hipMemcpyAsync( raw->dev, raw->host, off, hipMemcpyHostToDevice, ctx->copy ) );
  hipEvent_t up = get_event( ctx );
  HIP_TRY( hipEventRecord( up, ctx->copy ) );
  HIP_TRY( hipStreamWaitEvent( ps, up, 0 ) );
  { bool any_host = false; for ( int i = 0; i < n; i++ ) any_host = any_host || raw->items[i].on_host;
    if ( any_host ) HIP_TRY( hipStreamWaitEvent( ctx->tok.host_up, up, 0 ) ); }
  ctx->free_events.push_back( up );
  const aa::ParseJob * jobs_dev = reinterpret_cast<const aa::ParseJob *>( raw->dev );
  if ( n_order ) {
    LaunchTimer t( ctx, 3, ps );
    if ( int e = aa::launch_parse_mb_headers( jobs_dev, launch_order_dev, n_order, ps ) ) return hip_fail( static_cast<hipError_t>( e ), "k_parse_mb_headers" );
  }
  if ( n_seg_streams ) {
    if ( ctx->last_seg_batch ) HIP_TRY( hipStreamWaitEvent( ps, ctx->last_seg_batch, 0 ) );
    const uint8_t * segs_dev = raw->dev + jobs_bytes + dframes_bytes + sums_bytes;
    if ( int e = aa::launch_segment_fixup( jobs_dev, reinterpret_cast<const aa_seg_stream *>( segs_dev ), n_seg_streams,
                                           reinterpret_cast<const uint32_t *>( segs_dev + size_t( n ) * sizeof( aa_seg_stream ) ), ps ) )
      return hip_fail( static_cast<hipError_t>( e ), "k_segment_fixup" );
    if ( !ctx->last_seg_batch ) HIP_TRY( hipEventCreateWithFlags( &ctx->last_seg_batch, hipEventDisableTiming ) );
    HIP_TRY( hipEventRecord( ctx->last_seg_batch, ps ) );
  }
  raw->ps = ps; raw->launch_order_dev = launch_order_dev; raw->launch_order_host = launch_order; raw->n_order = n_order;
  raw->tokens_pending = true; raw->patch_jobs = defer_tokens;
  HIP_TRY( hipEventRecord( raw->hdr_done, ps ) );
  HIP_TRY( hipEventRecord( ctx->parse_idle[pick], ps ) );
  ctx->deferred.push_back( raw );
  abandon.armed = false;
  {
    int n_host = 0;
    for ( int i = 0; i < n; i++ ) if ( raw->items[i].on_host ) n_host++;
    if ( n_host ) {
      host_lanes_start( ctx );
      { std::lock_guard<std::mutex> g( ctx->host_lanes.mu );
        for ( int i = 0; i < n; i++ ) if ( raw->items[i].on_host ) { ctx->host_lanes.backlog_bytes += items[i].size; ctx->host_lanes.q.push_back( { raw, i } ); } }
      ctx->host_lanes.cv.notify_all();
      ctx->stats.host_routed_frames += static_cast<uint64_t>( n_host );
      if ( std::find( ctx->tok.inflight.begin(), ctx->tok.inflight.end(), raw ) == ctx->tok.inflight.end() ) ctx->tok.inflight.push_back( raw );
    }
  }
  if ( !defer_tokens ) if ( aa_status st = launch_tokens_of( ctx, raw ) ) return st;
  if ( first_error != AA_OK ) return fail( first_error, first_message );
  return AA_OK;
}

}
```

### alfalfa_amd/csrc/runtime_types.inc

```
namespace {

thread_local std::string g_last_error;


aa_status fail( aa_status code, const std::string & msg ) { g_last_error = msg; return code; }

int effective_cpus()
{
  static const int n = [] {
    int cpus = static_cast<int>( std::thread::hardware_concurrency() );
    if ( cpus < 1 ) cpus = 1;
    cpu_set_t set;
    if ( sched_getaffinity( 0, sizeof set, &set ) == 0 ) { const int a = CPU_COUNT( &set ); if ( a > 0 && a < cpus ) cpus = a; }
    auto read_two = []( const char * path, double * a, double * b ) -> int {
      FILE * f = std::fopen( path, "r" );
      if ( !f ) return 0;
      char first[64] = { 0 };
      int got = std::fscanf( f, "%63s %lf", first, b );
      std::fclose( f );
      if ( got < 1 ) return 0;
      if ( std::strcmp( first, "max" ) == 0 ) { *a = -1; return got; }
      *a = atof( first );
      return got;
    };
    double quota = -1, period = 100000;
    if ( read_two( "/sys/fs/cgroup/cpu.max", &quota, &period ) < 1 ) {
      double q = -1, dummy = 0;
      if ( read_two( "/sys/fs/cgroup/cpu/cpu.cfs_quota_us", &q, &dummy ) >= 1 ) { quota = q; double pp = 100000; if ( read_two( "/sys/fs/cgroup/cpu/cpu.cfs_period_us", &pp, &dummy ) >= 1 && pp > 0 ) period = pp; }
    }
    if ( quota > 0 && period > 0 ) { const int q = std::max( 1, static_cast<int>( quota / period + 0.5 ) ); if ( q < cpus ) cpus = q; }
    return cpus;
  }();
  return n;
}
int worker_threads( int asked )
{
  const int cap = std::max( 1, std::min( 256, 2 * effective_cpus() ) );
  return std::max( 1, std::min( asked > 0 ? asked : cap, cap ) );
}
aa_status hip_fail( hipError_t e, const char * what )
{
  return fail( e == hipErrorNoDevice || e == hipErrorInvalidDevice ? AA_ERR_NO_DEVICE : AA_ERR_HIP,
               std::string( what ) + ": " + hipGetErrorString( e ) );
}
#define HIP_TRY( expr ) do { hipError_t e__ = ( expr ); if ( e__ != hipSuccess ) return hip_fail( e__, #expr ); } while ( 0 )

constexpr size_t kChunkBytes = size_t( 64 ) << 20;
constexpr size_t kAlign = 256;
inline size_t align_up( size_t v, size_t a = kAlign ) { return ( v + a - 1 ) / a * a; }

struct Chunk {
  uint8_t * host = nullptr;
  uint8_t * dev = nullptr;
  size_t capacity = 0, used = 0, uploaded = 0;
  size_t pinned_bytes = 0;
  size_t dev_bytes = 0;
  int live_frames = 0;
};

struct Batch {
  uint8_t * host = nullptr, * dev = nullptr;
  size_t host_bytes = 0, dev_bytes = 0;
  int n = 0, live = 0;
  hipEvent_t hdr_done = nullptr;
  size_t summaries_off = 0;
  uint8_t * host_dev = nullptr;
  bool tokens_pending = false;
  bool patch_jobs = false;
  size_t head_bytes = 0;
  const uint32_t * launch_order_dev = nullptr;
  uint32_t * launch_order_host = nullptr;
  int n_order = 0;
  int max_mbw = 0, max_nparts = 1;
  hipStream_t ps = nullptr;
  int parse_stream_index = 0;
  struct Item { aa_stream * s; int frame; bool live; bool on_host = false; size_t data_off = 0; uint8_t * host_dense = nullptr; size_t host_dense_bytes = 0; };
  std::vector<Item> items;
};

struct Slot {
  uint8_t * dev = nullptr;
  bool shared = false;
  int refs = 0;
  bool hash_valid = false;
  uint64_t hash = 0;
};

struct FrameRec {
  aa_frame_header hdr;
  aa_dev_frame * host_job = nullptr;
  const aa_dev_frame * dev_job = nullptr;
  int out_slot = -1;
  int ref_after[3] = { -1, -1, -1 };
  std::vector<uint8_t> intra_diagonals;
  bool has_split = false;
  bool handle_held = true;
  int chunk = -1;
  Batch * batch = nullptr;
  int batch_item = -1;
  bool summary_pending = false;
  uint8_t * rec_block = nullptr;
  size_t rec_bytes = 0;
  bool rec_in_arena = false;
  const uint32_t * chunk_list = nullptr;
  aa_mb_info * dev_mbs = nullptr;
  const uint32_t * packed_pos = nullptr;
  volatile aa::FrameSummary * summary = nullptr;
  const aa::ParseJob * parse_job = nullptr;
  bool enqueued = false;
  uint32_t est_chunks = 0;
  bool chunks_returned = false;
  bool records_released = false;
  bool placed = false;
};

}

struct aa_parser { aa::Parser impl; aa_parser( uint16_t w, uint16_t h ) : impl( w, h ) {} };

struct aa_ctx {
  int device = 0;
  hipStream_t compute = nullptr, copy = nullptr;
  hipEvent_t upload_done = nullptr;
  std::atomic<int> refs { 1 };
  struct BindBuf { aa_raster_binding * host = nullptr, * dev = nullptr; size_t cap = 0; hipEvent_t done = nullptr; bool busy = false; };
  static constexpr int kBindBufs = 16;
  BindBuf bind_bufs[kBindBufs];
  int next_bind_buf = 0;
  struct HostLanes {
    struct Task { Batch * b; int item; };
    std::mutex mu; std::condition_variable cv;
    std::deque<Task> q;
    std::vector<std::thread> threads;
    bool stop = false;
    std::atomic<uint64_t> parsed_bytes { 0 }, parse_us { 0 }, backlog_bytes { 0 };
    uint64_t parse_us_mark = 0;
  } host_lanes;
  struct GatherBuf { aa_gather_job * host = nullptr, * dev = nullptr; size_t cap = 0; hipEvent_t done = nullptr, copied = nullptr; bool busy = false; };
  GatherBuf gather_bufs[kBindBufs];
  int next_gather_buf = 0;
  struct RgbBuf { uint8_t * host = nullptr, * dev = nullptr; size_t cap = 0; hipEvent_t done = nullptr, before = nullptr, after = nullptr; bool busy = false; };
  RgbBuf rgb_bufs[kBindBufs];
  int next_rgb_buf = 0;
  RgbBuf quality_bufs[kBindBufs];
  int next_quality_buf = 0;
  int row_handoff_by_kernel[2] = { 0, 0 };
  std::deque<int> downloads_in_flight;
// ... 113 lines not shown
```

### alfalfa_amd/csrc/tok_fsm.hh

```
#pragma once
#include <initializer_list>

#include "parse_common.hh"

namespace aa {

struct alignas( 16 ) V16 { uint32_t x, y, z, w; };
struct alignas( 8 ) V8 { uint32_t x, y; };

#if defined( __HIP_DEVICE_COMPILE__ )
#define AA_GLOBAL __attribute__( ( address_space( 1 ) ) )
#else
#define AA_GLOBAL
#endif

struct FrameSummary {
  uint32_t num_coeff_blocks;
  uint32_t num_intra_mbs;
  uint32_t has_split;
  uint32_t steps;
  uint32_t num_chunks;
  uint32_t status;
  uint32_t done;
  uint32_t packed_words;
};
enum : uint32_t { TOK_OK = 0, TOK_STEP_BOUND = 1, TOK_NO_MEMORY = 2,
                  TOK_HOST_FAILED = 3 };

#if defined( __HIP_DEVICE_COMPILE__ )
#define AA_AT_ADD( p, v ) __hip_atomic_fetch_add( ( p ), ( v ), __ATOMIC_RELAXED, __HIP_MEMORY_SCOPE_AGENT )
#define AA_AT_ADD_ACQ( p, v ) __hip_atomic_fetch_add( ( p ), ( v ), __ATOMIC_ACQUIRE, __HIP_MEMORY_SCOPE_AGENT )
#define AA_AT_ADD_REL( p, v ) __hip_atomic_fetch_add( ( p ), ( v ), __ATOMIC_RELEASE, __HIP_MEMORY_SCOPE_AGENT )
#define AA_AT_LOAD( p ) __hip_atomic_load( ( p ), __ATOMIC_RELAXED, __HIP_MEMORY_SCOPE_AGENT )
#define AA_AT_STORE( p, v ) __hip_atomic_store( ( p ), ( v ), __ATOMIC_RELAXED, __HIP_MEMORY_SCOPE_AGENT )
#define AA_NOW() wall_clock64()
#else
template <class T, class V> AA_HD inline T aa_host_add( T * p, V v ) { const T old = *p; *p = static_cast<T>( old + static_cast<T>( v ) ); return old; }
#define AA_AT_ADD( p, v ) aa::aa_host_add( ( p ), ( v ) )
#define AA_AT_ADD_ACQ( p, v ) aa::aa_host_add( ( p ), ( v ) )
#define AA_AT_ADD_REL( p, v ) aa::aa_host_add( ( p ), ( v ) )
#define AA_AT_LOAD( p ) ( *( p ) )
#define AA_AT_STORE( p, v ) ( *( p ) = ( v ) )
AA_HD inline unsigned long long aa_host_clock() { static unsigned long long t = 0; return t += 1000; }
#define AA_NOW() aa::aa_host_clock()
#endif

struct CoeffPool {
  int32_t avail;
  uint32_t head;
  uint32_t reserve, publish;
  uint32_t mask;
  uint32_t starving;
  uint32_t pad[2];
};
constexpr uint32_t kChunkBlocks = 2048;
constexpr uint32_t kNoChunk = 0xFFFFFFFFu;
constexpr uint32_t kMbBlocks = 26;
constexpr uint32_t kChunkWords = kChunkBlocks * 16u;
constexpr uint32_t kMbMaskSlots = 25u;
constexpr uint32_t kMbWords = kMbMaskSlots + 25u * 16u;
AA_HD constexpr uint32_t chunk_list_entries( uint32_t nmb, uint32_t lanes = 1 ) { return 2u + ( nmb + 75u ) / 76u + 2u * ( lanes - 1u ); }

struct TokQueue {
  uint32_t head, reserve, publish, mask;
};

struct Heap {
  AA_GLOBAL int16_t * base;
  AA_GLOBAL CoeffPool * pool;
  AA_GLOBAL uint32_t * ring;
};

struct alignas( 16 ) ParseJob {
  FrameParams fp;
  const uint8_t * data;
  uint32_t size, data_padded;
  uint32_t nmb, flags_padded;
  aa_mb_info * mbs;
  uint32_t * chunk_list;
  uint32_t mp_stride;
  uint32_t mp_pad;
  uint32_t * packed_pos;
  unsigned long long * intra_rows;
  uint8_t * mbflags;
  FrameSummary * summary;
};

AA_HD inline uint32_t mp_flag_index( const ParseJob & J, uint32_t row, uint32_t col )
{
  const uint32_t P = J.fp.nparts;
  return J.flags_padded + ( row % P ) * J.mp_stride + ( row / P ) * J.fp.mbw + col;
}
AA_HD constexpr uint32_t mp_flag_stride( uint32_t mbw, uint32_t mbh, uint32_t P ) { return ( ( ( mbh + P - 1u ) / P ) * mbw + 15u ) & ~15u; }

namespace tok {

constexpr uint32_t kPeriod = 32;
constexpr uint32_t kRing = 128;
constexpr uint32_t kChunks = 2;
constexpr uint32_t kMetaRing = 32;
constexpr uint32_t kMetaChunks = 1;
static_assert( kRing >= 3 * kPeriod && 16 * kChunks == kPeriod && ( kRing & ( kRing - 1 ) ) == 0, "stream ring invariant" );

constexpr uint32_t kNodeTabOff = 0;
constexpr uint32_t kBandTabOff = 384;
constexpr uint32_t kXtab = 408;
constexpr uint32_t kSignX = 26;
constexpr uint32_t kBlockTabOff = 440;
constexpr uint32_t kIdleTabOff = 648;
constexpr uint32_t kTablesBytes = 768;
AA_HD constexpr uint32_t ring_addr( uint32_t lane ) { return kTablesBytes + lane * 128u; }
AA_HD constexpr uint32_t slice_addr( uint32_t lane, uint32_t lanes, uint32_t lane_bytes ) { return kTablesBytes + lanes * 128u + lane * ( lane_bytes - 128u ); }
constexpr uint32_t kMeta = 0;
constexpr uint32_t kPlaneBytes = 264;
constexpr uint32_t kPlaneY = kMeta + kMetaRing;
constexpr uint32_t kPlaneUV = kPlaneY + kPlaneBytes;
constexpr uint32_t kPlaneY2 = kPlaneUV + kPlaneBytes;
constexpr uint32_t kAbove = kPlaneY2 + kPlaneBytes;
static_assert( kPlaneY % 8 == 0 && kPlaneUV % 8 == 0 && kPlaneY2 % 8 == 0 && kPlaneY2 / 8 < 128, "plane offsets travel as bytes / 8 in the block table" );
AA_HD constexpr uint32_t above_bytes( uint32_t mbw, bool shared ) { return shared ? 2u * mbw : mbw + ( mbw + 7u ) / 8u; }
AA_HD constexpr uint32_t part_off( uint32_t mbw, bool shared ) { return ( kAbove + above_bytes( mbw, shared ) + 15 ) & ~15u; }
AA_HD constexpr uint32_t lane_lds_bytes( uint32_t mbw, bool multi_partition, bool shared = false )
{
  return kRing + part_off( mbw, shared ) + ( multi_partition ? 128u : 0u );
}

constexpr uint8_t kXtabInit[27] = { 159, 165, 145, 173, 148, 140, 176, 155, 140, 135, 180, 157, 141, 134, 130,
                                    254, 254, 243, 230, 196, 177, 153, 140, 133, 130, 129, 128 };

enum : uint32_t { kNodes = 47, kIdleRecs = 5,
                  R_MBDONE = kIdleTabOff, R_MB = kIdleTabOff + 8, R_DONE = kIdleTabOff + 16,
                  R_PARK = kIdleTabOff + 24,
                  R_BEND = kIdleTabOff + 32 };
static_assert( kIdleTabOff >= 512 && R_BEND + 8 <= kTablesBytes && kNodes * 8 <= kBandTabOff, "node addresses below 512, idle records from 512 on" );
constexpr uint32_t H_ROWREL = 1u << 31, H_XS = 1u << 15, H_ADV = 1u << 16, H_EMIT = 1u << 17;
constexpr uint32_t kZeroX = 27;
constexpr uint32_t half_at( uint32_t next_addr, uint32_t pk, uint32_t flags, uint32_t ctx = 0, uint32_t addv = 0 )
{
  return next_addr | ( pk << 10 ) | flags | ( ( ctx * 11 ) << 19 ) | ( addv << 24 );
}
constexpr uint32_t half( uint32_t next, uint32_t pk, uint32_t flags, uint32_t ctx = 0, uint32_t addv = 0 ) { return half_at( next * 8, pk, flags, ctx, addv ); }
constexpr uint32_t tree( uint32_t k ) { return half( k, k, H_ROWREL ); }
constexpr uint32_t sign_node( uint32_t addv )
{
  return addv <= 4 ? 36 + addv : ( addv == 5 ? 41 : addv == 7 ? 42 : addv == 11 ? 43 : addv == 19 ? 44 : addv == 35 ? 45 : 46 );
}
constexpr uint32_t to_sign( uint32_t addv, uint32_t flags = 0 ) { return half( sign_node( addv ), kSignX, flags ); }
constexpr uint32_t to_extra( uint32_t e ) { return half( e, e - 11, 0 ); }
struct NodeTable { V8 n[kNodes]; };
constexpr NodeTable make_nodes()
{
  NodeTable t {};
  t.n[0] = { half_at( R_BEND, kZeroX, 0 ), tree( 1 ) };
  t.n[1] = { half( 1, 1, H_ROWREL | H_ADV ), tree( 2 ) };
  t.n[2] = { to_sign( 1 ), tree( 3 ) };
  t.n[3] = { tree( 4 ), tree( 6 ) };
  t.n[4] = { to_sign( 2 ), tree( 5 ) };
  t.n[5] = { to_sign( 3 ), to_sign( 4 ) };
  t.n[6] = { tree( 7 ), tree( 8 ) };
  t.n[7] = { to_extra( 11 ), to_extra( 12 ) };
  t.n[8] = { tree( 9 ), tree( 10 ) };
  t.n[9] = { to_extra( 14 ), to_extra( 17 ) };
  t.n[10] = { to_extra( 21 ), to_extra( 26 ) };
  const uint32_t first[6] = { 11, 12, 14, 17, 21, 26 }, last[6] = { 11, 13, 16, 20, 25, 36 }, base[6] = { 5, 7, 11, 19, 35, 67 };
  for ( uint32_t c = 0; c < 6; c++ )
    for ( uint32_t e = first[c]; e <= last[c]; e++ ) {
      const uint32_t h = e == last[c] ? to_sign( base[c], H_XS ) : ( to_extra( e + 1 ) | H_XS );
      t.n[e] = { h, h };
    }
  const uint32_t addvs[10] = { 1, 2, 3, 4, 5, 7, 11, 19, 35, 67 };
// ... 18 lines not shown
    t.b[blk] = { a | ( ( 16 + l ) << 8 ) | ( sel << 16 ) | ( bit << 24 ), ( 1u << a ) | ( 1u << ( 16 + l ) ) };
  }
  t.b[25] = { 0, 0 };
  return t;
}
constexpr BlockTable kBlockTable = make_blocks();
static_assert( kBandTabOff % 32 == 0 && kBandTabOff + 18 <= kXtab && kXtab + 28 <= kBlockTabOff && kBlockTabOff % 8 == 0 && kBlockTabOff + sizeof( BlockTable ) <= kIdleTabOff
               && kTablesBytes % 128 == 0, "tables overlap" );

constexpr uint64_t nib( std::initializer_list<unsigned> v ) { uint64_t r = 0; unsigned i = 0; for ( unsigned x : v ) r |= static_cast<uint64_t>( x ) << ( 4 * i++ ); return r; }
constexpr uint64_t kZigzagNib = nib( { 0, 1, 4, 8, 5, 2, 3, 6, 9, 12, 13, 10, 7, 11, 14, 15 } );
constexpr uint64_t kBandNib = nib( { 0, 1, 2, 3, 6, 4, 5, 6, 6, 6, 6, 6, 6, 6, 6, 7 } );

struct Frame {
  const AA_GLOBAL ParseJob * job;
  const AA_GLOBAL uint8_t * data;
  const AA_GLOBAL uint8_t * mbflags;
  AA_GLOBAL aa_mb_info * mbs;
  AA_GLOBAL uint32_t * chunk_list;
  AA_GLOBAL uint32_t * packed_pos;
  uint32_t data_padded, flags_padded, nmb, mbw, nparts;
  uint32_t max_steps;
  uint32_t mp_P, mp_p;
  uint32_t mp_owner;
};
AA_HD inline Frame frame_of( const ParseJob * job )
{
  Frame F;
  F.job = (const AA_GLOBAL ParseJob *) job;
  F.data = (const AA_GLOBAL uint8_t *) job->data; F.mbflags = (const AA_GLOBAL uint8_t *) job->mbflags;
  F.mbs = (AA_GLOBAL aa_mb_info *) job->mbs; F.chunk_list = (AA_GLOBAL uint32_t *) job->chunk_list;
  F.packed_pos = (AA_GLOBAL uint32_t *) job->packed_pos;
  const uint64_t bound = static_cast<uint64_t>( job->nmb ) * ( 25u * ( 16u * 23u + 8u ) + 8u ) + 4096u;
  F.max_steps = bound > 0xFFFFFFF0ull ? 0xFFFFFFF0u : static_cast<uint32_t>( bound );
  F.data_padded = job->data_padded; F.flags_padded = job->flags_padded; F.nmb = job->nmb; F.mbw = job->fp.mbw; F.nparts = job->fp.nparts;
  F.mp_P = 1; F.mp_p = 0; F.mp_owner = 0;
  return F;
}
AA_HD inline Frame frame_of_partition( const ParseJob * job, uint32_t p, uint32_t owner_base )
{
  Frame F = frame_of( job );
  const uint32_t P = job->fp.nparts, mbh = job->fp.mbh;
  const uint32_t rows = mbh > p ? ( mbh - p + P - 1u ) / P : 0u;
  F.mbflags = (const AA_GLOBAL uint8_t *) job->mbflags + job->flags_padded + p * job->mp_stride;
  F.nmb = rows * F.mbw;
  F.flags_padded = job->mp_stride;
  F.mp_P = P; F.mp_p = p; F.mp_owner = owner_base;
  return F;
}
AA_HD inline uint32_t mp_owner_partition( const ParseJob * job ) { return ( job->fp.mbh - 1u ) % job->fp.nparts; }

struct MpDeal { uint32_t ticket, part, n, start; bool any; };
template <class PartsOf>
AA_HD inline MpDeal mp_deal( uint32_t n_idle, uint32_t got, uint32_t rank, PartsOf parts_of )
{
  MpDeal d { 0, 0, 1, 0, false };
  uint32_t spare = n_idle - got, start = 0;
  for ( uint32_t t = 0; t < got; t++ ) {
    const uint32_t P = parts_of( t );
    const uint32_t n = ( P > 1u && P - 1u <= spare ) ? P : 1u;
    spare -= n - 1u;
    if ( rank >= start && rank < start + n ) { d.ticket = t; d.part = rank - start; d.n = n; d.start = start; d.any = true; }
    start += n;
  }
  return d;
}

struct MpShared {
  uint32_t prog[8];
  uint32_t nchunks;
  uint32_t left;
  uint32_t blocks, words, steps;
  uint32_t status;
};
static_assert( sizeof( MpShared ) <= 128, "MpShared lives in the partition save area" );

struct Chunk16 { uint32_t w[4]; };

AA_HD inline Chunk16 load16( const AA_GLOBAL uint8_t * p )
{
  const AA_GLOBAL V16 * q = (const AA_GLOBAL V16 *) p;
  const V16 v = *q;
  Chunk16 c; c.w[0] = v.x; c.w[1] = v.y; c.w[2] = v.z; c.w[3] = v.w;
  return c;
}
AA_HD inline void lds_store16( uint8_t * smem, uint32_t off, const Chunk16 & c )
{
  V16 v; v.x = c.w[0]; v.y = c.w[1]; v.z = c.w[2]; v.w = c.w[3];
  *reinterpret_cast<V16 *>( smem + off ) = v;
}
AA_HD inline Chunk16 mask_past_end( Chunk16 c, uint32_t at, uint32_t end )
{
  for ( uint32_t k = 0; k < 4; k++ ) {
    const uint32_t a = at + 4 * k;
    const uint32_t keep = a >= end ? 0u : ( end - a >= 4 ? 0xFFFFFFFFu : ( ( 1u << ( 8 * ( end - a ) ) ) - 1u ) );
    c.w[k] &= keep;
  }
  return c;
}

struct Lane {
  uint32_t base;
  uint32_t sbase;
  uint32_t value, range;
  int32_t sh;
  uint32_t rpos, rend;
  uint32_t wpos;
  uint32_t mwpos;
  uint32_t pend_wpos, pend_mwpos;
  Chunk16 pend[kChunks], mpend[kMetaChunks];
  uint32_t rec;
  uint32_t pre_prob, pre_raw, pre_band;
  V8 pre_rec;
  uint32_t paddr;
  uint32_t rowaddr, typeaddr;
  uint32_t ia;
  uint32_t mag, nonzero;
  uint32_t blkaddr;
  uint32_t nzsel, blkbit;
  uint32_t blkslot;
  uint32_t ctxbits;
  uint32_t flags, nz_mask, mb_first, coeff_blocks, yfirst;
  uint32_t ykind;
  uint32_t y2byte;
  uint32_t nx_mi;
  uint32_t nx_flags, nx_above, nx_y2;
  AA_GLOBAL int16_t * blk;
  uint32_t blk_index;
  uint32_t blk_left;
  uint32_t nchunks;
  unsigned long long mem_since;
  AA_GLOBAL int16_t * sink;
  AA_GLOBAL int16_t * hdr;
  uint32_t zzmask;
  uint32_t words;
  uint32_t mi_real;
  uint32_t chunk_ord;
  uint32_t mi, col, row, part;
  uint32_t steps;
};
constexpr uint32_t kNoPend = 0xFFFFFFFFu;
constexpr uint32_t kNoPlane = 0xFFFFFFFFu;

AA_HD inline void zero_slot( AA_GLOBAL int16_t * block )
{
  V16 z; z.x = z.y = z.z = z.w = 0;
  AA_GLOBAL V16 * p = (AA_GLOBAL V16 *) block;
  p[0] = z; p[1] = z;
}

AA_HD inline uint32_t pool_take( const Heap & H )
{
  const int32_t old = AA_AT_ADD( &H.pool->avail, -1 );
  if ( old <= 0 ) { AA_AT_ADD( &H.pool->avail, 1 ); return kNoChunk; }
  const uint32_t t = AA_AT_ADD( &H.pool->head, 1u );
  return AA_AT_LOAD( &H.ring[t & H.pool->mask] );
}
AA_HD inline void pool_push( const Heap & H, const AA_GLOBAL uint32_t * ids, uint32_t first, uint32_t n )
{
  if ( !n ) return;
  const uint32_t b = AA_AT_ADD( &H.pool->reserve, n );
  for ( uint32_t i = 0; i < n; i++ ) AA_AT_STORE( &H.ring[( b + i ) & H.pool->mask], ids ? ids[i] : first + i );
  while ( AA_AT_LOAD( &H.pool->publish ) != b ) {}
  AA_AT_STORE( &H.pool->publish, b + n );
  AA_AT_ADD_REL( &H.pool->avail, static_cast<int32_t>( n ) );
}

AA_HD inline void prime_stream( Lane & L, uint8_t * smem, const Frame & J )
{
  const uint32_t base = L.rpos & ~15u;
  for ( uint32_t k = 0; k < kRing / 16; k++ ) {
    const uint32_t at = base + 16 * k;
    Chunk16 c; c.w[0] = c.w[1] = c.w[2] = c.w[3] = 0;
    if ( at < J.data_padded ) c = load16( J.data + at );
    lds_store16( smem, L.sbase + ( at & ( kRing - 1 ) ), mask_past_end( c, at, L.rend ) );
  }
  L.wpos = base + kRing;
  L.pend_wpos = kNoPend;
}

AA_HD inline void start_partition( Lane & L, uint8_t * smem, const Frame & J, uint32_t p )
{
  L.part = p;
  L.rpos = J.job->fp.part_off[p];
  L.rend = J.job->fp.part_off[p] + J.job->fp.part_size[p];
  prime_stream( L, smem, J );
  uint32_t v = 0;
  for ( int k = 0; k < 4; k++ ) { v = ( v << 8 ) | smem[L.sbase + ( L.rpos & ( kRing - 1 ) )]; L.rpos++; }
  L.value = v; L.sh = -8; L.range = 255;
}

template <bool SH = false>
AA_HD inline void switch_partition( Lane & L, uint8_t * smem, const Frame & J, uint32_t p )
{
  const uint32_t save = L.base + part_off( J.mbw, SH );
  uint32_t * s = reinterpret_cast<uint32_t *>( smem + save + 16 * L.part );
  s[0] = L.value; s[1] = L.range | ( static_cast<uint32_t>( L.sh + 64 ) << 8 ); s[2] = L.rpos; s[3] = 1;
  const uint32_t * t = reinterpret_cast<const uint32_t *>( smem + save + 16 * p );
  if ( !t[3] ) { start_partition( L, smem, J, p ); return; }
  L.part = p;
  L.value = t[0]; L.range = t[1] & 255u; L.sh = static_cast<int32_t>( t[1] >> 8 ) - 64; L.rpos = t[2];
  L.rend = J.job->fp.part_off[p] + J.job->fp.part_size[p];
  prime_stream( L, smem, J );
}

template <bool MP = false>
AA_HD inline void top_up( Lane & L, uint8_t * smem, const Frame & J )
{
  if ( L.rec == R_DONE || ( MP && L.rec == R_PARK ) ) return;
  if ( L.pend_wpos == L.wpos ) {
    for ( uint32_t k = 0; k < kChunks; k++ )
      lds_store16( smem, L.sbase + ( ( L.wpos + 16 * k ) & ( kRing - 1 ) ), mask_past_end( L.pend[k], L.wpos + 16 * k, L.rend ) );
    L.wpos += 16 * kChunks;
  }
  if ( L.pend_mwpos == L.mwpos ) {
    for ( uint32_t k = 0; k < kMetaChunks; k++ ) lds_store16( smem, L.base + kMeta + ( ( L.mwpos + 16 * k ) & ( kMetaRing - 1 ) ), L.mpend[k] );
    L.mwpos += 16 * kMetaChunks;
  }
  L.pend_wpos = L.pend_mwpos = kNoPend;
  if ( L.wpos - L.rpos <= kRing - 16 * kChunks ) {
    for ( uint32_t k = 0; k < kChunks; k++ ) {
      const uint32_t at = L.wpos + 16 * k;
      Chunk16 c; c.w[0] = c.w[1] = c.w[2] = c.w[3] = 0;
      if ( at < J.data_padded ) c = load16( J.data + at );
      L.pend[k] = c;
    }
    L.pend_wpos = L.wpos;
  }
  if ( L.mwpos - L.mi <= kMetaRing - 16 * kMetaChunks ) {
    for ( uint32_t k = 0; k < kMetaChunks; k++ ) {
      const uint32_t at = L.mwpos + 16 * k;
      Chunk16 c; c.w[0] = c.w[1] = c.w[2] = c.w[3] = 0;
      if ( at < J.flags_padded ) c = load16( J.mbflags + at );
      L.mpend[k] = c;
    }
    L.pend_mwpos = L.mwpos;
  }
}

#if defined( __HIP_DEVICE_COMPILE__ )
#define AA_ANY( x ) ( __builtin_amdgcn_ballot_w64( x ) != 0 )
#define AA_LDS_ADD( smem, off, v ) __hip_atomic_fetch_add( aa::tok::lds_at<uint32_t>( ( smem ), ( off ) ), ( v ), __ATOMIC_RELAXED, __HIP_MEMORY_SCOPE_WORKGROUP )
#define AA_LDS_LOAD( smem, off ) __hip_atomic_load( aa::tok::lds_at<uint32_t>( ( smem ), ( off ) ), __ATOMIC_RELAXED, __HIP_MEMORY_SCOPE_WORKGROUP )
#define AA_MUL24( a, b ) __umul24( ( a ), ( b ) )
#define AA_POPC( v ) static_cast<uint32_t>( __builtin_popcount( v ) )
#define AA_UBFE( v, off, width ) __builtin_amdgcn_ubfe( ( v ), ( off ), ( width ) )
#define AA_BFI( m, a, b ) ( ( ( m ) & ( a ) ) | ( ~( m ) & ( b ) ) )
#define AA_SBFE( v, off, width ) __builtin_amdgcn_sbfe( static_cast<int>( v ), ( off ), ( width ) )
#define AA_CLZ( v ) __builtin_clz( v )
template <class T> __device__ inline __attribute__( ( address_space( 3 ) ) ) T * lds_at( uint8_t *, uint32_t off )
{
  return (__attribute__( ( address_space( 3 ) ) ) T *) static_cast<uintptr_t>( off );
}
#else
#define AA_ANY( x ) ( x )
#define AA_LDS_ADD( smem, off, v ) aa::aa_host_add( aa::tok::lds_at<uint32_t>( ( smem ), ( off ) ), ( v ) )
#define AA_LDS_LOAD( smem, off ) ( *aa::tok::lds_at<uint32_t>( ( smem ), ( off ) ) )
#define AA_MUL24( a, b ) ( ( a ) * ( b ) )
#define AA_POPC( v ) static_cast<uint32_t>( __builtin_popcount( v ) )
#define AA_UBFE( v, off, width ) ( ( ( v ) >> ( off ) ) & ( ( 1u << ( width ) ) - 1u ) )
#define AA_BFI( m, a, b ) ( ( ( m ) & ( a ) ) | ( ~( m ) & ( b ) ) )
#define AA_SBFE( v, off, width ) ( static_cast<int32_t>( static_cast<uint32_t>( v ) << ( 32 - ( off ) - ( width ) ) ) >> ( 32 - ( width ) ) )
#define AA_CLZ( v ) ( ( v ) ? __builtin_clz( v ) : 32 )
template <class T> inline T * lds_at( uint8_t * smem, uint32_t off ) { return reinterpret_cast<T *>( smem + off ); }
#endif

AA_HD inline void store_mb( const Frame & J, uint32_t mi, uint32_t nz_mask, uint32_t coeff_index, uint32_t flags )
{
  AA_GLOBAL aa_mb_info * mb = J.mbs + mi;
  mb->nz_mask = nz_mask;
  mb->coeff_index = coeff_index;
  mb->flags = static_cast<uint8_t>( flags );
}

AA_HD inline void store_mb_packed( const Frame & J, uint32_t mi, uint32_t nz_mask, uint32_t pos, uint32_t flags, unsigned long long word_off = 0 )
{
  AA_GLOBAL aa_mb_info * mb = J.mbs + mi;
  mb->nz_mask = nz_mask;
  mb->coeff_index = static_cast<uint32_t>( word_off );
  mb->flags = static_cast<uint8_t>( flags );
  mb->reserved = static_cast<uint8_t>( word_off >> 32 );
  J.packed_pos[mi] = pos;
}

AA_HD inline void preload( Lane & L, uint8_t * smem )
{
  L.pre_prob = *lds_at<const uint8_t>( smem, L.paddr );
  L.pre_raw = *lds_at<const uint8_t>( smem, L.sbase | ( L.rpos & ( kRing - 1 ) ) );
  L.pre_rec = *lds_at<const V8>( smem, L.rec );
  L.pre_band = *lds_at<const uint8_t>( smem, L.ia + 1u );
}

AA_HD inline AA_GLOBAL int16_t * bump_words( AA_GLOBAL int16_t * p, uint32_t n )
{
#if defined( __HIP_DEVICE_COMPILE__ )
  const unsigned long long a = reinterpret_cast<unsigned long long>( p );
  return reinterpret_cast<AA_GLOBAL int16_t *>( ( a & 0xFFFFFFFF00000000ull ) | static_cast<uint32_t>( static_cast<uint32_t>( a ) + 2u * n ) );
#else
  return p + n;
#endif
}

AA_HD inline void setup_first_block( Lane & L, uint32_t has_y2 )
{
  constexpr V8 e0 = kBlockTable.b[0], e1 = kBlockTable.b[1];
  static_assert( ( ( e0.x >> 16 ) & 255u ) == kPlaneY2 / 8 && ( ( e1.x >> 16 ) & 255u ) == kPlaneY / 8 + kBlkIsY, "first blocks: Y2 / Y" );
  const bool y2 = has_y2 != 0u;
  L.blkaddr = kBlockTabOff + ( y2 ? 8u : 16u );
  L.nzsel = y2 ? e0.y : e1.y;
  L.blkslot = y2 ? e0.x >> 24 : e1.x >> 24;
  L.blkbit = 1u << L.blkslot;
  const uint32_t ctx = AA_POPC( L.ctxbits & L.nzsel );
  L.typeaddr = L.base + ( y2 ? kPlaneY2 : kPlaneY );
  L.ia = kBandTabOff;
  L.rowaddr = L.typeaddr + ctx * 11u;
  L.rec = 0; L.paddr = L.rowaddr;
// ... 33 lines not shown
  AA_LDS_ADD( smem, sh + offsetof( MpShared, words ), words );
  AA_LDS_ADD( smem, sh + offsetof( MpShared, steps ), L.steps );
  L.blk = L.sink;
  const uint32_t left = AA_LDS_ADD( smem, sh + offsetof( MpShared, left ), 0xFFFFFFFFu );
  L.rec = ( left != 1u && L.base == J.mp_owner ) ? static_cast<uint32_t>( R_PARK ) : static_cast<uint32_t>( R_DONE );
  if ( left != 1u ) return;
  const MpShared fin = *lds_at<const MpShared>( smem, sh );
  J.chunk_list[0] = fin.nchunks;
  AA_GLOBAL FrameSummary * sum = (AA_GLOBAL FrameSummary *) J.job->summary;
  sum->num_coeff_blocks = fin.blocks;
  sum->packed_words = PK ? fin.words : 0u;
  sum->steps = fin.steps;
  sum->num_chunks = fin.nchunks;
  sum->status = fin.status;
#if defined( __HIP_DEVICE_COMPILE__ )
  __builtin_amdgcn_fence( __ATOMIC_RELEASE, "" );
  asm volatile( "s_waitcnt vmcnt(0)" ::: "memory" );
  __hip_atomic_store( &sum->done, 1u, __ATOMIC_RELAXED, __HIP_MEMORY_SCOPE_SYSTEM );
#else
  sum->done = 1u;
#endif
}

template <bool SH>
AA_HD inline uint32_t above_load( uint8_t * smem, uint32_t abase, uint32_t mbw, uint32_t col, uint32_t & y2byte )
{
  if constexpr ( SH ) return *lds_at<const uint16_t>( smem, abase + 2u * col );
  else {
    const uint32_t yuv = *lds_at<const uint8_t>( smem, abase + col );
    y2byte = *lds_at<const uint8_t>( smem, abase + mbw + ( col >> 3 ) );
    return yuv | ( ( ( y2byte >> ( col & 7u ) ) & 1u ) << 8 );
  }
}
template <bool SH>
AA_HD inline void above_store( uint8_t * smem, uint32_t abase, uint32_t mbw, uint32_t col, uint32_t bits, uint32_t & y2byte )
{
  if constexpr ( SH ) *lds_at<uint16_t>( smem, abase + 2u * col ) = static_cast<uint16_t>( bits );
  else {
    *lds_at<uint8_t>( smem, abase + col ) = static_cast<uint8_t>( bits );
    const uint32_t m = 1u << ( col & 7u );
    y2byte = ( bits & 0x100u ) ? y2byte | m : y2byte & ~m;
    *lds_at<uint8_t>( smem, abase + mbw + ( col >> 3 ) ) = static_cast<uint8_t>( y2byte );
  }
}

template <uint32_t ROUNDS = 1>
AA_HD inline void load_plane( uint8_t * smem, uint32_t at, const Frame & J, uint32_t type )
{
  constexpr uint32_t per = kPlaneBytes / 4 / ROUNDS;
  static_assert( per * ROUNDS * 4 == kPlaneBytes, "whole rounds" );
  const AA_GLOBAL uint32_t * src = (const AA_GLOBAL uint32_t *) &J.job->fp.coeff_probs[type][0][0][0];
  auto dst = lds_at<uint32_t>( smem, at );
  if constexpr ( ROUNDS == 1 ) { for ( uint32_t k = 0; k < per; k++ ) dst[k] = src[k]; }
  else {
    _Pragma( "unroll 1" )
    for ( uint32_t r = 0; r < ROUNDS; r++ )
      for ( uint32_t k = 0; k < per; k++ ) dst[r * per + k] = src[r * per + k];
  }
}

constexpr unsigned long long kMemWaitTicks = 200000000ull;

template <bool PK, bool MP = false>
AA_HD inline void macroblock_boundary_body( Lane & L, uint8_t * smem, const Frame & J, const Heap & H )
{
  const bool mp = MP && J.mp_P > 1;
  const uint32_t above = ( mp ? J.mp_owner : L.base ) + kAbove;
  const uint32_t shared = J.mp_owner + part_off( J.mbw, true );
  if constexpr ( MP ) if ( L.rec == R_PARK ) {
    if ( AA_LDS_LOAD( smem, shared + offsetof( MpShared, left ) ) == 0u ) L.rec = R_DONE;
    return;
  }
  if ( L.rec == R_MBDONE ) {
    above_store<MP>( smem, above, J.mbw, L.col, L.ctxbits, L.y2byte );
    L.mi++; L.col++; L.rec = R_MB;
    if constexpr ( MP ) { L.mi_real++; if ( mp ) *lds_at<uint32_t>( smem, shared + 4 * J.mp_p ) = L.mi; }
  }
  enum : uint32_t { V_WAIT = 0, V_CODED = 1, V_FINISH = 2, V_SWITCH = 3 };
  uint32_t verdict = V_WAIT, flags = 0, status = TOK_OK;
  if ( L.steps > J.max_steps ) { verdict = V_FINISH; status = TOK_STEP_BOUND; }
  else for ( ;; ) {
    if constexpr ( MP ) if ( mp && AA_LDS_LOAD( smem, shared + offsetof( MpShared, status ) ) != TOK_OK ) { verdict = V_FINISH; break; }
    if ( L.mi == J.nmb ) { verdict = V_FINISH; break; }
    if ( L.mi >= L.mwpos ) break;
    if ( L.col == J.mbw ) {
      L.col = 0; L.row++; L.ctxbits = 0;
      if constexpr ( MP ) if ( mp ) L.mi_real += ( J.mp_P - 1u ) * J.mbw;
      if ( !mp && J.nparts > 1 ) { verdict = V_SWITCH; break; }
    }
    if constexpr ( MP ) if ( mp && ( J.mp_p | L.row ) != 0 ) {
      const uint32_t q = J.mp_p ? J.mp_p - 1u : J.mp_P - 1u, k = J.mp_p ? L.row : L.row - 1u;
      if ( AA_LDS_LOAD( smem, shared + 4 * q ) < k * J.mbw + L.col + 1u ) break;
    }
    uint32_t up;
    if ( !MP && L.nx_mi == L.mi ) {
      flags = L.nx_flags;
      L.y2byte = ( L.col & 7u ) ? L.y2byte : L.nx_y2;
      up = L.nx_above | ( ( ( L.y2byte >> ( L.col & 7u ) ) & 1u ) << 8 );
    } else {
      flags = smem[L.base + kMeta + ( L.mi & ( kMetaRing - 1 ) )];
      up = above_load<MP>( smem, above, J.mbw, L.col, L.y2byte );
    }
    L.ctxbits = ( L.ctxbits & 0x01FF0000u ) | up;
    if ( !( flags & AA_MB_SKIP ) ) { verdict = V_CODED; break; }
    const uint32_t has_y2 = flags & AA_MB_HAS_Y2;
    L.ctxbits &= has_y2 ? 0u : 0x01000100u;
    above_store<MP>( smem, above, J.mbw, L.col, L.ctxbits, L.y2byte );
    const uint32_t mi_rec = MP ? L.mi_real : L.mi;
    if constexpr ( PK ) store_mb_packed( J, mi_rec, 0, 0, flags | ( has_y2 ? AA_MB_LF_SKIP_INNER : 0u ) );
    else store_mb( J, mi_rec, 0, L.blk_index, flags | ( has_y2 ? AA_MB_LF_SKIP_INNER : 0u ) );
    L.mi++; L.col++;
    if constexpr ( MP ) { L.mi_real++; if ( mp ) *lds_at<uint32_t>( smem, shared + 4 * J.mp_p ) = L.mi; }
  }
  if ( verdict == V_WAIT ) return;
  if ( verdict == V_SWITCH ) { switch_partition<MP>( L, smem, J, L.row % J.nparts ); return; }
  if ( verdict == V_FINISH ) {
    if ( mp ) finish_partition<PK>( L, smem, J, H, status );
    else finish_frame<PK>( L, J, H, status );
    return;
  }
  const uint32_t has_y2 = flags & AA_MB_HAS_Y2;
  const uint32_t used = PK && L.nchunks ? static_cast<uint32_t>( L.blk - ( H.base + static_cast<size_t>( L.blk_index ) * 16 ) ) : 0u;
  if ( PK ? ( !L.nchunks || used + kMbWords + 1u > kChunkWords ) : L.blk_left < kMbBlocks ) {
    const uint32_t c = pool_take( H );
    if ( c == kNoChunk ) {
      const unsigned long long now = AA_NOW();
      if ( !L.mem_since ) { L.mem_since = now | 1ull; AA_AT_ADD( &H.pool->starving, 1u ); }
      else if ( now - L.mem_since > kMemWaitTicks ) { if ( mp ) finish_partition<PK>( L, smem, J, H, TOK_NO_MEMORY ); else finish_frame<PK>( L, J, H, TOK_NO_MEMORY ); }
      return;
    }
    L.mem_since = 0;
    if ( mp ) {
      L.chunk_ord = AA_LDS_ADD( smem, shared + offsetof( MpShared, nchunks ), 1u );
      J.chunk_list[1 + L.chunk_ord] = c;
    } else {
      J.chunk_list[1 + L.nchunks] = c;
      if constexpr ( MP ) L.chunk_ord = L.nchunks;
    }
    L.nchunks++;
    L.blk_index = c * kChunkBlocks;
    if constexpr ( PK ) {
      L.words += used;
      L.blk = H.base + static_cast<size_t>( L.blk_index ) * 16;
    } else {
      L.blk = H.base + static_cast<size_t>( L.blk_index ) * 16;
      L.blk_left = kChunkBlocks;
      zero_slot( L.blk );
    }
  }
  if constexpr ( PK ) {
    L.mb_first = ( ( MP ? L.chunk_ord : L.nchunks - 1u ) << 15 ) | static_cast<uint32_t>( L.blk - ( H.base + static_cast<size_t>( L.blk_index ) * 16 ) );
    L.hdr = L.blk; L.blk = L.hdr + kMbMaskSlots; L.zzmask = 0;
  } else L.mb_first = L.blk_index;
  L.flags = flags; L.nz_mask = 0;
  const uint32_t kind = has_y2 ? Y_AFTER_Y2 : Y_WITHOUT_Y2;
  if ( L.ykind != kind ) { load_plane<PK ? 1 : 2>( smem, L.base + kPlaneY, J, kind ); L.ykind = kind; }
  L.yfirst = has_y2 ? 1u : 0u;
  setup_first_block( L, has_y2 );
}

template <bool PK, bool MP = false>
AA_HD inline void macroblock_boundary( Lane & L, uint8_t * smem, const Frame & J, const Heap & H )
{
  macroblock_boundary_body<PK, MP>( L, smem, J, H );
  preload( L, smem );
}

// ... 53 lines not shown
  const int16_t coeff = static_cast<int16_t>( bit ? -m : m );
  if constexpr ( PK ) {
    *( emit ? L.blk : L.sink ) = coeff;
    L.blk = bump_words( L.blk, emit );
    L.zzmask |= emit << ( pos & 31u );
  } else {
    const uint32_t zz = static_cast<uint32_t>( kZigzagNib >> ( ( pos & 15u ) * 4 ) ) & 15u;
    if ( emit ) L.blk[zz] = coeff;
    L.nonzero |= emit;
  }
  L.mag = emit ? 0u : mag;
}

template <bool PK, bool MP = false>
AA_HD inline void block_end( Lane & L, uint8_t * smem, const Frame & J, const Heap & H )
{
  (void) H;
  if ( L.rec == R_BEND ) {
    const V8 nextblk = *lds_at<const V8>( smem, L.blkaddr );
    const bool nonzero = PK ? L.zzmask != 0 : L.nonzero != 0;
    const uint32_t ctxbits = nonzero ? L.ctxbits | L.nzsel : L.ctxbits & ~L.nzsel;
    if constexpr ( PK ) {
      if ( nonzero ) { L.coeff_blocks++; L.hdr[L.blkslot] = static_cast<int16_t>( L.zzmask ); L.zzmask = 0; L.nz_mask |= L.blkbit; }
    } else {
      if ( nonzero ) { L.coeff_blocks++; L.blk += 16; L.blk_index++; L.blk_left--; zero_slot( L.blk ); L.nz_mask |= L.blkbit; }
    }
    const bool mbdone = L.blkaddr == kBlockTabOff + 8 * 25;
    if ( mbdone ) {
      uint32_t flags = L.flags;
      flags |= L.nz_mask ? AA_MB_HAS_NONZERO : ( ( flags & AA_MB_HAS_Y2 ) ? AA_MB_LF_SKIP_INNER : 0u );
      if constexpr ( PK ) {
        store_mb_packed( J, MP ? L.mi_real : L.mi, L.nz_mask, L.mb_first, flags, static_cast<unsigned long long>( L.hdr - H.base ) );
        if ( !L.nz_mask ) L.blk = L.hdr;
      } else store_mb( J, MP ? L.mi_real : L.mi, L.nz_mask, L.mb_first, flags );
      if constexpr ( !MP ) {
        const uint32_t nmi = L.mi + 1u, ncol = L.col + 1u;
        const bool ok = nmi < L.mwpos && ncol < J.mbw;
        const uint32_t c = ok ? ncol : 0u;
        L.nx_flags = *lds_at<const uint8_t>( smem, L.base + kMeta + ( nmi & ( kMetaRing - 1 ) ) );
        L.nx_above = *lds_at<const uint8_t>( smem, L.base + kAbove + c );
        L.nx_y2 = *lds_at<const uint8_t>( smem, L.base + kAbove + J.mbw + ( c >> 3 ) );
        L.nx_mi = ok ? nmi : kNoPend;
      }
    }
    const uint32_t sel = AA_UBFE( nextblk.x, 16, 8 );
    const uint32_t nctx = AA_POPC( ctxbits & nextblk.y );
    L.typeaddr = L.base + 8u * ( sel & ( kBlkIsY - 1u ) );
    const uint32_t idx = ( sel >> 7 ) & L.yfirst;
    L.ia = kBandTabOff + idx;
    L.rowaddr = L.paddr = L.typeaddr + idx * 33u + nctx * 11u;
    L.ctxbits = ctxbits;
    L.blkaddr += 8;
    L.nzsel = nextblk.y;
    L.blkslot = nextblk.x >> 24;
    L.blkbit = 1u << L.blkslot;
    L.nonzero = 0; L.mag = 0;
    L.rec = mbdone ? static_cast<uint32_t>( R_MBDONE ) : 0u;
    preload( L, smem );
  }
}

struct PeriodProf { unsigned long long pass_ticks, passes, steps; };
template <bool PK, bool MP = false>
AA_HD inline void run_period( Lane & L, uint8_t * smem, const Frame & J, const Heap & H, bool prof, PeriodProf & P )
{
  uint32_t it = 0;
  while ( it < kPeriod ) {
    if ( AA_ANY( at_boundary<MP>( L ) ) ) {
      const unsigned long long tb = prof ? AA_NOW() : 0ull;
      if ( at_boundary<MP>( L ) ) macroblock_boundary<PK, MP>( L, smem, J, H );
      if ( prof ) { P.pass_ticks += AA_NOW() - tb; P.passes++; }
      it++;
      if ( !AA_ANY( L.rec < R_MBDONE ) ) break;
    }
    const uint32_t it0 = it;
    do {
#pragma unroll
      for ( uint32_t k = 0; k < kBendEvery; k++ ) step<PK, MP>( L, smem, J );
      it += kBendEvery;
      if ( AA_ANY( L.rec == R_BEND ) ) block_end<PK, MP>( L, smem, J, H );
    } while ( it < kPeriod && !AA_ANY( L.rec == R_MBDONE ) );
    if ( prof ) P.steps += it - it0;
  }
  if ( L.rec != R_DONE ) L.steps += it;
}
template <bool PK, bool MP = false>
AA_HD inline void run_period( Lane & L, uint8_t * smem, const Frame & J, const Heap & H )
{
  PeriodProf none { 0, 0, 0 };
  run_period<PK, MP>( L, smem, J, H, false, none );
}

AA_HD inline uint32_t table_word( uint32_t k )
{
  const uint32_t * n = reinterpret_cast<const uint32_t *>( &kNodeTable );
  const uint32_t * b = reinterpret_cast<const uint32_t *>( &kBlockTable );
  if ( k < sizeof( NodeTable ) / 4 ) return n[k];
  if ( k >= kBlockTabOff / 4 && k < ( kBlockTabOff + sizeof( BlockTable ) ) / 4 ) return b[k - kBlockTabOff / 4];
  if ( k >= kIdleTabOff / 4 && k < kIdleTabOff / 4 + 2 * kIdleRecs ) return idle_half( ( k - kIdleTabOff / 4 ) / 2 );
  if ( k >= kBandTabOff / 4 && k < kBandTabOff / 4 + 5 ) {
    uint32_t w = 0;
    for ( uint32_t i = 0; i < 4; i++ ) { const uint32_t at = 4 * ( k - kBandTabOff / 4 ) + i; w |= ( at < 16 ? 33u * ( static_cast<uint32_t>( kBandNib >> ( 4 * at ) ) & 15u ) : 0u ) << ( 8 * i ); }
    return w;
  }
  if ( k >= kXtab / 4 && k < kXtab / 4 + 7 ) {
    uint32_t w = 0;
    for ( uint32_t i = 0; i < 4; i++ ) { const uint32_t at = 4 * ( k - kXtab / 4 ) + i; w |= ( at < 27 ? static_cast<uint32_t>( kXtabInit[at] ) : 0u ) << ( 8 * i ); }
    return w;
  }
  return 0;
}

AA_HD inline void init_lane( Lane & L, uint32_t sbase, uint32_t base, AA_GLOBAL int16_t * sink )
{
  L.sink = sink;
  L.sbase = sbase; L.base = base;
  L.rec = R_DONE; L.paddr = kXtab + kZeroX; L.ia = kBandTabOff; L.rowaddr = L.typeaddr = base;
  L.value = 0; L.range = 255; L.sh = 0; L.rpos = 0; L.mag = 0; L.zzmask = 0; L.nonzero = 0;
  L.blk = sink; L.hdr = nullptr;
  L.pend_wpos = L.pend_mwpos = kNoPend;
  L.y2byte = 0; L.nx_mi = kNoPend; L.nx_flags = L.nx_above = L.nx_y2 = 0;
  L.steps = 0;
}

template <bool SH = false>
AA_HD inline void begin_frame( Lane & L, uint8_t * smem, uint32_t base, const Frame & J )
{
  L.base = base;
  uint8_t * lds = smem + base;
  load_plane<3>( smem, base + kPlaneUV, J, UV );
  load_plane<3>( smem, base + kPlaneY2, J, Y2 );
  L.ykind = kNoPlane;
  if ( J.nparts > 1 ) for ( uint32_t k = 0; k < 128 / 4; k++ ) reinterpret_cast<uint32_t *>( lds + part_off( J.mbw, SH ) )[k] = 0;
  for ( uint32_t k = 0; k < above_bytes( J.mbw, SH ); k++ ) lds[kAbove + k] = 0;
  L.mi = 0; L.col = 0; L.row = 0; L.ctxbits = 0; L.coeff_blocks = 0; L.steps = 0;
  L.flags = L.nz_mask = L.mb_first = L.yfirst = 0;
  L.nonzero = L.nzsel = L.blkbit = L.blkslot = L.mag = 0;
  L.ia = kBandTabOff;
  L.typeaddr = L.rowaddr = base; L.paddr = kXtab + kZeroX;
  L.blkaddr = kBlockTabOff;
  L.blk = L.sink; L.blk_index = 0; L.blk_left = 0; L.nchunks = 0; L.mem_since = 0;
  L.hdr = nullptr; L.zzmask = 0; L.words = 0;
  L.mi_real = 0; L.chunk_ord = 0;
  L.y2byte = 0; L.nx_mi = kNoPend;
  if ( J.mp_P > 1 ) {
    L.mi_real = J.mp_p * J.mbw;
    if ( base == J.mp_owner ) {
      MpShared z {};
      z.left = J.mp_P;
      *reinterpret_cast<MpShared *>( lds + part_off( J.mbw, SH ) ) = z;
    }
  }
  start_partition( L, smem, J, J.mp_P > 1 ? J.mp_p : 0u );
  for ( uint32_t k = 0; k < kMetaRing / 16; k++ ) {
    Chunk16 c; c.w[0] = c.w[1] = c.w[2] = c.w[3] = 0;
    if ( 16 * k < J.flags_padded ) c = load16( J.mbflags + 16 * k );
    lds_store16( smem, base + kMeta + 16 * k, c );
  }
  L.mwpos = kMetaRing;
  L.pend_mwpos = kNoPend;
  L.rec = R_MB;
  preload( L, smem );
}

}
}
```

### include/alfalfa_amd.h

```cpp
#ifndef ALFALFA_AMD_H
#define ALFALFA_AMD_H

#include <stddef.h>
#include <stdint.h>

#ifdef __cplusplus
extern "C" {
#endif

#define AA_ABI_VERSION 4

typedef enum aa_status {
  AA_OK = 0,
  AA_ERR_INVALID = -1,
  AA_ERR_UNSUPPORTED = -2,
  AA_ERR_LOGIC = -3,
  AA_ERR_OUT_OF_RANGE = -4,
  AA_ERR_HIP = -5,
  AA_ERR_NO_DEVICE = -6,
  AA_ERR_ARGUMENT = -7,
  AA_ERR_NO_MEMORY = -8
} aa_status;

const char * aa_last_error( void );
// ... 140 lines not shown
int aa_stream_error_concealment( const aa_stream * s );

int aa_stream_frame_count( const aa_stream * s );
aa_status aa_stream_release_before( aa_stream * s, int first_kept );
aa_status aa_stream_rewind( aa_stream * s );
aa_status aa_stream_rewind_to( aa_stream * s, int frame_index );

aa_status aa_stream_download( aa_stream * s, int frame_index, uint8_t * y, uint8_t * u, uint8_t * v );
aa_status aa_pinned_alloc( aa_ctx * ctx, size_t bytes, void ** out );
void aa_pinned_free( void * p );
aa_status aa_stream_download_async( aa_stream * s, int frame_index, uint8_t * y, uint8_t * u, uint8_t * v );
aa_status aa_stream_download_wait( aa_stream * s );
aa_status aa_download_batch_async( aa_ctx * ctx, aa_stream * const * streams, int n, const int * frame_index, uint8_t * dst, size_t stride );
aa_status aa_ctx_download_wait( aa_ctx * ctx );
aa_status aa_ctx_download_wait_until( aa_ctx * ctx, int max_in_flight );
aa_status aa_stream_raster_device( aa_stream * s, int frame_index, void ** y, void ** u, void ** v );
enum { AA_RGB_U8_HWC3 = 0, AA_RGB_U8_HWC4 = 1, AA_RGB_U8_CHW = 2, AA_RGB_F16_CHW = 3, AA_RGB_BF16_CHW = 4, AA_RGB_F32_CHW = 5 };
typedef struct aa_rgb_target { void * dst; int64_t row_stride; int64_t plane_stride; } aa_rgb_target;
aa_status aa_render_rgb_async( aa_ctx * ctx, aa_stream * const * streams, int n, const int * frame_index, int format,
                               const aa_rgb_target * targets, const double mean[3], const double std[3], void * consumer_stream );
enum { AA_QUALITY_Y = 1, AA_QUALITY_YUV = 3 };
typedef struct aa_quality_ref { const void * y, * u, * v; int64_t y_stride, uv_stride; } aa_quality_ref;
aa_status aa_quality_batch_async( aa_ctx * ctx, aa_stream * const * streams, int n, const int * frame_index,
                                  const aa_quality_ref * originals, int planes,
                                  double * ssim_dev, uint64_t * sse_dev, void * consumer_stream );
aa_status aa_stream_references( const aa_stream * s, int * last, int * golden, int * alternate );
aa_status aa_stream_reference_slots( const aa_stream * s, int slots[3] );
aa_status aa_stream_import_reference( aa_stream * s, const void * y_dev, const void * u_dev, const void * v_dev );
aa_status aa_stream_import_reference_host( aa_stream * s, const uint8_t * y, const uint8_t * u, const uint8_t * v );

aa_status aa_stream_export_raster( aa_stream * s, int frame_index, void * y_dev, void * u_dev, void * v_dev );
size_t aa_stream_state_size( const aa_stream * s );
aa_status aa_stream_export_state( const aa_stream * s, uint8_t * buf, size_t capacity );
aa_status aa_stream_import_state( aa_stream * s, const uint8_t * buf, size_t size );

aa_status aa_stream_serialize( aa_stream * s, uint8_t * buf, size_t capacity, size_t * size );
aa_status aa_stream_deserialize( aa_stream * s, const uint8_t * buf, size_t size );

aa_status aa_parser_state_hash( const aa_parser * p, uint64_t * out );
aa_status aa_stream_state_hash( aa_stream * s, uint64_t * out );
aa_status aa_stream_raster_hash( aa_stream * s, int frame_index, uint64_t * out );
aa_status aa_stream_decoder_hash( aa_stream * s, uint64_t parts[4], uint64_t * whole );
aa_status aa_stream_minihash( aa_stream * s, uint32_t * out );
aa_status aa_stream_release_frame( aa_stream * s, int frame_index );
aa_status aa_stream_set_references( aa_stream * s, const void * const planes[3][3], const int is_host[3] );
aa_status aa_stream_reference_device( aa_stream * s, int which, void ** y, void ** u, void ** v );
aa_status aa_stream_reference_download( aa_stream * s, int which, uint8_t * y, uint8_t * u, uint8_t * v );

void aa_raster_geometry( uint16_t width, uint16_t height, uint32_t * padded_width, uint32_t * padded_height );

aa_status aa_stream_lf_search( aa_stream * s, const uint8_t * data, size_t size, const uint8_t * original_luma,
                               int level_lo, int level_hi, int * best_level, double * best_ssim, double * ssim_out, uint8_t * rasters_out );

aa_status aa_ssim_host( const uint8_t * a, const uint8_t * b, int width, int height, double * out );

typedef struct aa_kernel_stats {
  double recon_inter_ms, recon_intra_ms, loopfilter_ms;
  uint64_t recon_inter_launches, recon_intra_launches, loopfilter_launches;
  uint64_t macroblocks;
  double parse_headers_ms, parse_tokens_ms;
  uint64_t parse_launches;
  uint64_t parsed_macroblocks;
  double recon_split_ms;
  uint64_t recon_split_launches;
  uint64_t pool_waits;
  double pool_wait_ms, parse_wait_ms;
  double bind_wait_ms;
  double alloc_ms;
  uint64_t slab_mallocs;
  uint64_t token_steps;
  uint64_t token_frames;
  uint64_t worker_launches, worker_wgs;
  uint64_t worker_retires;
  uint64_t heap_grows;
  uint64_t heap_mapped_bytes;
  uint64_t nomem_retries;
  uint64_t frames_evicted;
  uint64_t host_routed_frames;
  uint64_t row_handoff_stale_polls;
  uint64_t row_handoff_rereads;
  uint64_t packed_frames, packed_words, packed_blocks;
  double host_batch_ms, host_batch_parse_wall_ms, host_batch_parse_cpu_ms, host_batch_arena_ms;
  uint64_t pinned_allocs;
} aa_kernel_stats;
aa_status aa_ctx_profile( aa_ctx * ctx, int enable );
aa_status aa_ctx_kernel_stats( aa_ctx * ctx, aa_kernel_stats * out, int reset );

#ifdef __cplusplus
}
#endif
#endif
```

Measured before the change: 126.0 million.

## Overlap token parsing with macroblock header parsing via row progress handoff

The header-parse kernel now publishes a per-frame row-progress word and, after the first two rows, enqueues the frame's job directly into the token queue. Token workers start early, read macroblock flags with agent-scope atomic loads, and stall whenever flags for the next chunk are not yet written. The goal is to hide header-parse latency behind token decoding instead of waiting for the whole header pass and a separate enqueue kernel. In exchange it adds polling, per-row fences and a timeout error path, and it is on by default unless disabled by an environment variable.

```diff
diff --git a/alfalfa_amd/capi.py b/alfalfa_amd/capi.py
--- a/alfalfa_amd/capi.py
+++ b/alfalfa_amd/capi.py
@@ -49,7 +49,7 @@
                 ("worker_retires", C.c_uint64), ("heap_grows", C.c_uint64), ("heap_mapped_bytes", C.c_uint64), ("nomem_retries", C.c_uint64), ("frames_evicted", C.c_uint64), ("host_routed_frames", C.c_uint64),
                 ("row_handoff_stale_polls", C.c_uint64), ("row_handoff_rereads", C.c_uint64), ("packed_frames", C.c_uint64), ("packed_words", C.c_uint64), ("packed_blocks", C.c_uint64),
                 ("host_batch_ms", C.c_double), ("host_batch_parse_wall_ms", C.c_double), ("host_batch_parse_cpu_ms", C.c_double), ("host_batch_arena_ms", C.c_double),
-                ("pinned_allocs", C.c_uint64)]
+                ("pinned_allocs", C.c_uint64), ("token_header_waits", C.c_uint64)]
 
 
 class CtxInfo(C.Structure):
diff --git a/alfalfa_amd/csrc/device_types.h b/alfalfa_amd/csrc/device_types.h
--- a/alfalfa_amd/csrc/device_types.h
+++ b/alfalfa_amd/csrc/device_types.h
@@ -80,12 +80,13 @@
   uint32_t pool_starving;
   uint32_t exited[AA_MAX_WORKER_GRIDS];
   unsigned long long prof[8];
+  uint32_t hdr_waits;
 };
 
 namespace aa {
 struct ParseJob;
 struct TokQueue; struct CoeffPool; struct Heap;
-int launch_parse_mb_headers( const ParseJob * jobs, const uint32_t * order, int n, void * stream );
+int launch_parse_mb_headers( const ParseJob * jobs, const uint32_t * order, int n, void * stream, TokQueue * q = nullptr, unsigned long long * slots = nullptr, uint32_t delay_ticks = 0 );
 int launch_segment_fixup( const ParseJob * jobs, const aa_seg_stream * streams, int n_streams, const uint32_t * order, void * stream );
 void token_worker_shape( uint32_t lane_bytes, int n_cus, int * lanes_out, uint32_t * lds_out, int * wgs_per_cu_out );
 int launch_token_workers( TokQueue * q, unsigned long long * slots, const Heap & heap, uint32_t * exited, const uint32_t * retire, uint32_t gen, uint32_t spread,
diff --git a/alfalfa_amd/csrc/parse_kernels.hip b/alfalfa_amd/csrc/parse_kernels.hip
--- a/alfalfa_amd/csrc/parse_kernels.hip
+++ b/alfalfa_amd/csrc/parse_kernels.hip
@@ -14,7 +14,8 @@
 
 using aa::ParseJob;
 
-__global__ __launch_bounds__( 64 ) void k_parse_mb_headers( const ParseJob * jobs, const uint32_t * order, int n, int lanes )
+__global__ __launch_bounds__( 64 ) void k_parse_mb_headers( const ParseJob * jobs, const uint32_t * order, int n, int lanes,
+                                                            aa::TokQueue * q, unsigned long long * slots, uint32_t delay_ticks )
 {
   __builtin_amdgcn_s_setprio( 2 );
 
@@ -43,20 +44,51 @@
   uint32_t intra = 0, split = 0;
   unsigned mi = 0;
   const uint32_t mp_stride = J.mp_stride, mp_base = J.flags_padded, nparts = fp.nparts;
-  for ( unsigned row = 0; row < mbh; row++ ) {
-    unsigned long long word = 0;
-    const uint32_t mp_row = mp_stride ? mp_base + ( row % nparts ) * mp_stride + ( row / nparts ) * mbw : 0u;
-    for ( unsigned col = 0; col < mbw; col++, mi++ ) {
-      const uint8_t flags = aa::parse_mb_header( bd, fp, T, J.mbs, mi, col, row, static_cast<uint8_t *>( nullptr ) );
-      J.mbflags[mi] = flags;
-      if ( mp_stride ) J.mbflags[mp_row + col] = flags;
-      if ( !( flags & AA_MB_INTER ) ) { intra++; word |= 1ull << ( col & 63 ); }
-      else if ( J.mbs[mi].y_mode == aa::SPLITMV ) split = 1;
-      if ( ( col & 63 ) == 63 || col + 1 == mbw ) { J.intra_rows[row * words_per_row + ( col >> 6 )] = word; word = 0; }
-    }
-  }
-  J.summary->num_intra_mbs = intra;
-  J.summary->has_split = split;
+  const uint32_t q_mask = q ? q->mask : 0u;
+  uint32_t * const progress = const_cast<uint32_t *>( &Jp->hdr_rows );
+  const uint32_t lead = mbh < aa::kHdrLeadRows ? mbh : aa::kHdrLeadRows;
+  for ( unsigned row = 0; __any( row < mbh ); row++ ) {
+    const bool on = row < mbh;
+    if ( on ) {
+      if ( delay_ticks ) {
+        const unsigned long long t0 = wall_clock64();
+        for ( uint32_t k = 0; k < ( 1u << 22 ) && wall_clock64() - t0 < delay_ticks; k++ ) __builtin_amdgcn_s_sleep( 32 );
+      }
+      unsigned long long word = 0;
+      const uint32_t mp_row = mp_stride ? mp_base + ( row % nparts ) * mp_stride + ( row / nparts ) * mbw : 0u;
+      for ( unsigned col = 0; col < mbw; col++, mi++ ) {
+        const uint8_t flags = aa::parse_mb_header( bd, fp, T, J.mbs, mi, col, row, static_cast<uint8_t *>( nullptr ) );
+        J.mbflags[mi] = flags;
+        if ( mp_stride ) J.mbflags[mp_row + col] = flags;
+        if ( !( flags & AA_MB_INTER ) ) { intra++; word |= 1ull << ( col & 63 ); }
+        else if ( J.mbs[mi].y_mode == aa::SPLITMV ) split = 1;
+        if ( ( col & 63 ) == 63 || col + 1 == mbw ) { J.intra_rows[row * words_per_row + ( col >> 6 )] = word; word = 0; }
+      }
+      if ( row + 1 == mbh ) { J.summary->num_intra_mbs = intra; J.summary->has_split = split; }
+    }
+    if ( !q ) continue;
+    __builtin_amdgcn_fence( __ATOMIC_RELEASE, "" );
+    asm volatile( "s_waitcnt vmcnt(0)" ::: "memory" );
+    if ( on ) __hip_atomic_store( progress, row + 1 == mbh ? aa::kHdrDone : row + 2, __ATOMIC_RELAXED, __HIP_MEMORY_SCOPE_AGENT );
+    const bool hand_over = on && row + 1 == lead;
+    const unsigned long long givers = __ballot( hand_over );
+    if ( givers ) {
+      const int first = __ffsll( static_cast<long long>( givers ) ) - 1;
+      const uint32_t cnt = static_cast<uint32_t>( __popcll( givers ) );
+      uint32_t base = 0;
+      if ( lane == first ) base = AA_AT_ADD( &q->reserve, cnt );
+      base = __shfl( base, first );
+      const uint32_t rank = static_cast<uint32_t>( __popcll( givers & ( ( 1ull << lane ) - 1ull ) ) );
+      if ( hand_over ) AA_AT_STORE( &slots[( base + rank ) & q_mask], reinterpret_cast<unsigned long long>( Jp ) );
+      __builtin_amdgcn_fence( __ATOMIC_RELEASE, "agent" );
+      asm volatile( "s_waitcnt vmcnt(0)" ::: "memory" );
+      if ( lane == first ) {
+        while ( AA_AT_LOAD( &q->publish ) != base ) __builtin_amdgcn_s_sleep( 8 );
+        AA_AT_STORE( &q->publish, base + cnt );
+      }
+    }
+  }
+  if ( !q ) { J.summary->num_intra_mbs = intra; J.summary->has_split = split; }
 }
 
 __global__ __launch_bounds__( 256 ) void k_segment_fixup( const ParseJob * jobs, const aa_seg_stream * streams, const uint32_t * order )
@@ -302,7 +334,7 @@
   if ( threadIdx.x || blockIdx.x ) return;
   if ( prof ) for ( int k = 0; k < 8; k++ ) out->prof[k] = AA_AT_LOAD( &prof[k] );
   out->q_head = AA_AT_LOAD( &q->head ); out->q_publish = AA_AT_LOAD( &q->publish ); out->q_reserve = AA_AT_LOAD( &q->reserve );
-  if ( pool ) { out->pool_avail = AA_AT_LOAD( &pool->avail ); out->pool_starving = AA_AT_LOAD( &pool->starving ); }
+  if ( pool ) { out->pool_avail = AA_AT_LOAD( &pool->avail ); out->pool_starving = AA_AT_LOAD( &pool->starving ); out->hdr_waits = AA_AT_LOAD( &pool->hdr_waits ); }
   for ( int g = 0; g < n_grids; g++ ) out->exited[g] = AA_AT_LOAD( &exited[g] );
   __builtin_amdgcn_fence( __ATOMIC_RELEASE, "" );
   asm volatile( "s_waitcnt vmcnt(0)" ::: "memory" );
@@ -340,10 +372,10 @@
   return { 0, 0, 0 };
 }
 
-int launch_parse_mb_headers( const ParseJob * jobs, const uint32_t * order, int n, void * stream )
+int launch_parse_mb_headers( const ParseJob * jobs, const uint32_t * order, int n, void * stream, TokQueue * q, unsigned long long * slots, uint32_t delay_ticks )
 {
   const int lanes = header_lanes();
-  hipLaunchKernelGGL( k_parse_mb_headers, dim3( ( n + lanes - 1 ) / lanes ), dim3( 64 ), 0, static_cast<hipStream_t>( stream ), jobs, order, n, lanes );
+  hipLaunchKernelGGL( k_parse_mb_headers, dim3( ( n + lanes - 1 ) / lanes ), dim3( 64 ), 0, static_cast<hipStream_t>( stream ), jobs, order, n, lanes, q, slots, delay_ticks );
   return static_cast<int>( hipGetLastError() );
 }
 
diff --git a/alfalfa_amd/csrc/runtime_ctx.inc b/alfalfa_amd/csrc/runtime_ctx.inc
--- a/alfalfa_amd/csrc/runtime_ctx.inc
+++ b/alfalfa_amd/csrc/runtime_ctx.inc
@@ -371,6 +371,10 @@
   for ( auto ps : ctx->parse_streams ) HIP_TRY( hipStreamSynchronize( ps ) );
   drain_profile( ctx );
   ctx->stats.heap_mapped_bytes = ctx->tok.heap_mapped;
+  if ( ctx->tok.ready ) {
+    if ( aa_status st = tok_refresh_mirror( ctx ) ) return st;
+    ctx->stats.token_header_waits = ctx->tok.mirror_host->hdr_waits;
+  }
   if ( ctx->ws ) {
     int rescued[6] = {};
     HIP_TRY( hipMemcpy( rescued, &ctx->ws->dump[AA_SYNC_WS_RESCUES], sizeof rescued, hipMemcpyDeviceToHost ) );
diff --git a/alfalfa_amd/csrc/runtime_decode.inc b/alfalfa_amd/csrc/runtime_decode.inc
--- a/alfalfa_amd/csrc/runtime_decode.inc
+++ b/alfalfa_amd/csrc/runtime_decode.inc
@@ -65,6 +65,9 @@
     if ( aa_status st = tok_service( ctx ) ) return st;
   }
   if ( sum->status == aa::TOK_HOST_FAILED ) return fail( AA_ERR_HIP, "host lane: the frame's records could not be placed in device memory" );
+  if ( ( sum->status & 255u ) == aa::TOK_HEADER_WAIT )
+    return fail( AA_ERR_HIP, "device parser: the token lane of frame " + std::to_string( static_cast<int>( &r - s->frames.data() ) ) + " (" + std::to_string( r.hdr.mb_width ) + " x " + std::to_string( r.hdr.mb_height )
+                             + " macroblocks) waited more than half a second for macroblock row " + std::to_string( sum->status >> 8 ) + " of its header pass (k_parse_mb_headers) and gave up (records are not valid)" );
   if ( sum->status == aa::TOK_STEP_BOUND ) return fail( AA_ERR_HIP, "device parser: a token lane exceeded the step bound of its frame size (records are not valid)" );
   r.hdr.num_coeff_blocks = sum->num_coeff_blocks;
   r.hdr.num_intra_mbs = sum->num_intra_mbs;
diff --git a/alfalfa_amd/csrc/runtime_records.inc b/alfalfa_amd/csrc/runtime_records.inc
--- a/alfalfa_amd/csrc/runtime_records.inc
+++ b/alfalfa_amd/csrc/runtime_records.inc
@@ -39,6 +39,7 @@
       ctx->tok.inflight.erase( std::remove( ctx->tok.inflight.begin(), ctx->tok.inflight.end(), b ), ctx->tok.inflight.end() );
       ctx->tok.batches.erase( std::remove( ctx->tok.batches.begin(), ctx->tok.batches.end(), b ), ctx->tok.batches.end() );
       if ( b->hdr_done ) { (void) hipEventSynchronize( b->hdr_done ); (void) hipEventDestroy( b->hdr_done ); }
+      if ( b->hdr_start ) (void) hipEventDestroy( b->hdr_start );
       { std::lock_guard<std::mutex> g( ctx->pool_mu ); ctx->pinned_pool.emplace_back( b->host, b->host_bytes ); }
       dev_free( ctx, b->dev, b->dev_bytes, true );
       delete b;
diff --git a/alfalfa_amd/csrc/runtime_submit.inc b/alfalfa_amd/csrc/runtime_submit.inc
--- a/alfalfa_amd/csrc/runtime_submit.inc
+++ b/alfalfa_amd/csrc/runtime_submit.inc
@@ -161,7 +161,8 @@
 
   J.data = b->dev + it.data_off;
   J.size = static_cast<uint32_t>( it.size ); J.data_padded = ( J.size + 15u ) & ~15u;
-  J.nmb = nmb; J.flags_padded = flags_padded; J.mp_stride = mp_stride; J.mp_pad = 0;
+  J.nmb = nmb; J.flags_padded = flags_padded; J.mp_stride = mp_stride;
+  J.hdr_rows = aa::kHdrDone;
   J.mbs = reinterpret_cast<aa_mb_info *>( blk );
   J.intra_rows = reinterpret_cast<unsigned long long *>( blk + mb_bytes );
   J.mbflags = blk + mb_bytes + rows_bytes;
@@ -195,16 +196,22 @@
 }
 
 namespace {
+aa_status tok_queue_room( aa_ctx * ctx, int n )
+{
+  auto & T = ctx->tok;
+  if ( static_cast<uint32_t>( T.jobs_enqueued ) - T.mirror_host->q_head + static_cast<uint32_t>( n ) + 4096u > T.q_slots ) {
+    if ( aa_status st = tok_refresh_mirror( ctx ) ) return st;
+    if ( static_cast<uint32_t>( T.jobs_enqueued ) - T.mirror_host->q_head + static_cast<uint32_t>( n ) + 4096u > T.q_slots )
+      if ( aa_status st = tok_quiesce( ctx ) ) return st;
+  }
+  return AA_OK;
+}
 aa_status launch_tokens_of( aa_ctx * ctx, Batch * b )
 {
   if ( !b->tokens_pending ) return AA_OK;
   auto & T = ctx->tok;
   aa::ParseJob * jobs_host = reinterpret_cast<aa::ParseJob *>( b->host );
-  if ( static_cast<uint32_t>( T.jobs_enqueued ) - T.mirror_host->q_head + static_cast<uint32_t>( b->n ) + 4096u > T.q_slots ) {
-    if ( aa_status st = tok_refresh_mirror( ctx ) ) return st;
-    if ( static_cast<uint32_t>( T.jobs_enqueued ) - T.mirror_host->q_head + static_cast<uint32_t>( b->n ) + 4096u > T.q_slots )
-      if ( aa_status st = tok_quiesce( ctx ) ) return st;
-  }
+  if ( !b->self_enqueue ) if ( aa_status st = tok_queue_room( ctx, b->n ) ) return st;
   b->tokens_pending = false;
   ctx->deferred.erase( std::remove( ctx->deferred.begin(), ctx->deferred.end(), b ), ctx->deferred.end() );
   bool dropped = false;
@@ -238,13 +245,14 @@
     if ( keep ) HIP_TRY( hipMemcpyAsync( const_cast<uint32_t *>( b->launch_order_dev ), b->launch_order_host, size_t( keep ) * sizeof( uint32_t ), hipMemcpyHostToDevice, ps ) );
   }
   if ( b->n_order > 0 ) {
-    if ( int e = aa::launch_enqueue_jobs( T.q, T.slots, reinterpret_cast<const aa::ParseJob *>( b->dev ), b->launch_order_dev, b->n_order, ps ) )
-      return hip_fail( static_cast<hipError_t>( e ), "k_enqueue_jobs" );
+    if ( !b->self_enqueue )
+      if ( int e = aa::launch_enqueue_jobs( T.q, T.slots, reinterpret_cast<const aa::ParseJob *>( b->dev ), b->launch_order_dev, b->n_order, ps ) )
+        return hip_fail( static_cast<hipError_t>( e ), "k_enqueue_jobs" );
     T.jobs_enqueued += static_cast<uint64_t>( b->n_order );
   }
   HIP_TRY( hipEventRecord( b->hdr_done, ps ) );
   HIP_TRY( hipEventRecord( ctx->parse_idle[b->parse_stream_index], ps ) );
-  return tok_service( ctx, b->hdr_done );
+  return tok_service( ctx, b->self_enqueue ? b->hdr_start : b->hdr_done );
 }
 }
 
@@ -602,6 +610,16 @@
   std::stable_sort( launch_order, launch_order + n_order, [&]( uint32_t a, uint32_t b ) { return items[a].size > items[b].size; } );
   const uint32_t * launch_order_dev = reinterpret_cast<const uint32_t *>( raw->dev + ( reinterpret_cast<uint8_t *>( launch_order ) - raw->host ) );
 
+  const char * overlap_env = std::getenv( "ALFALFA_AMD_HEADER_OVERLAP" );
+  const bool self_enqueue = !defer_tokens && n_order > 0 && n_seg_streams == 0 && !ctx->tok.lane_per_partition && !( overlap_env && atoi( overlap_env ) == 0 );
+  uint32_t hdr_delay_ticks = 0;
+  if ( const char * e = std::getenv( "ALFALFA_AMD_HEADER_ROW_DELAY_US" ) ) hdr_delay_ticks = static_cast<uint32_t>( std::max( 0, std::min( 2000000, atoi( e ) ) ) ) * 100u;
+  if ( self_enqueue ) {
+    if ( aa_status st = tok_queue_room( ctx, n ) ) return st;
+    for ( int i = 0; i < n_order; i++ ) jobs_host[launch_order[i]].hdr_rows = 1;
+    raw->self_enqueue = true;
+  }
+
   HIP_TRY( hipEventCreateWithFlags( &raw->hdr_done, hipEventDisableTiming ) );
   HIP_TRY( hipMemcpyAsync( raw->dev, raw->host, off, hipMemcpyHostToDevice, ctx->copy ) );
   hipEvent_t up = get_event( ctx );
@@ -612,8 +630,13 @@
   ctx->free_events.push_back( up );
   const aa::ParseJob * jobs_dev = reinterpret_cast<const aa::ParseJob *>( raw->dev );
   if ( n_order ) {
+    if ( self_enqueue ) {
+      HIP_TRY( hipEventCreateWithFlags( &raw->hdr_start, hipEventDisableTiming ) );
+      HIP_TRY( hipEventRecord( raw->hdr_start, ps ) );
+    }
     LaunchTimer t( ctx, 3, ps );
-    if ( int e = aa::launch_parse_mb_headers( jobs_dev, launch_order_dev, n_order, ps ) ) return hip_fail( static_cast<hipError_t>( e ), "k_parse_mb_headers" );
+    if ( int e = aa::launch_parse_mb_headers( jobs_dev, launch_order_dev, n_order, ps, self_enqueue ? ctx->tok.q : nullptr, ctx->tok.slots, hdr_delay_ticks ) )
+      return hip_fail( static_cast<hipError_t>( e ), "k_parse_mb_headers" );
   }
   if ( n_seg_streams ) {
     if ( ctx->last_seg_batch ) HIP_TRY( hipStreamWaitEvent( ps, ctx->last_seg_batch, 0 ) );
diff --git a/alfalfa_amd/csrc/runtime_types.inc b/alfalfa_amd/csrc/runtime_types.inc
--- a/alfalfa_amd/csrc/runtime_types.inc
+++ b/alfalfa_amd/csrc/runtime_types.inc
@@ -63,6 +63,8 @@
   size_t host_bytes = 0, dev_bytes = 0;
   int n = 0, live = 0;
   hipEvent_t hdr_done = nullptr;
+  bool self_enqueue = false;
+  hipEvent_t hdr_start = nullptr;
   size_t summaries_off = 0;
   uint8_t * host_dev = nullptr;
   bool tokens_pending = false;
diff --git a/alfalfa_amd/csrc/tok_fsm.hh b/alfalfa_amd/csrc/tok_fsm.hh
--- a/alfalfa_amd/csrc/tok_fsm.hh
+++ b/alfalfa_amd/csrc/tok_fsm.hh
@@ -25,7 +25,8 @@
   uint32_t packed_words;
 };
 enum : uint32_t { TOK_OK = 0, TOK_STEP_BOUND = 1, TOK_NO_MEMORY = 2,
-                  TOK_HOST_FAILED = 3 };
+                  TOK_HOST_FAILED = 3,
+                  TOK_HEADER_WAIT = 4 };
 
 #if defined( __HIP_DEVICE_COMPILE__ )
 #define AA_AT_ADD( p, v ) __hip_atomic_fetch_add( ( p ), ( v ), __ATOMIC_RELAXED, __HIP_MEMORY_SCOPE_AGENT )
@@ -33,6 +34,7 @@
 #define AA_AT_ADD_REL( p, v ) __hip_atomic_fetch_add( ( p ), ( v ), __ATOMIC_RELEASE, __HIP_MEMORY_SCOPE_AGENT )
 #define AA_AT_LOAD( p ) __hip_atomic_load( ( p ), __ATOMIC_RELAXED, __HIP_MEMORY_SCOPE_AGENT )
 #define AA_AT_STORE( p, v ) __hip_atomic_store( ( p ), ( v ), __ATOMIC_RELAXED, __HIP_MEMORY_SCOPE_AGENT )
+#define AA_AT_LOAD_G( p ) __hip_atomic_load( ( p ), __ATOMIC_RELAXED, __HIP_MEMORY_SCOPE_AGENT )
 #define AA_NOW() wall_clock64()
 #else
 template <class T, class V> AA_HD inline T aa_host_add( T * p, V v ) { const T old = *p; *p = static_cast<T>( old + static_cast<T>( v ) ); return old; }
@@ -41,6 +43,7 @@
 #define AA_AT_ADD_REL( p, v ) aa::aa_host_add( ( p ), ( v ) )
 #define AA_AT_LOAD( p ) ( *( p ) )
 #define AA_AT_STORE( p, v ) ( *( p ) = ( v ) )
+#define AA_AT_LOAD_G( p ) ( *( p ) )
 AA_HD inline unsigned long long aa_host_clock() { static unsigned long long t = 0; return t += 1000; }
 #define AA_NOW() aa::aa_host_clock()
 #endif
@@ -51,7 +54,8 @@
   uint32_t reserve, publish;
   uint32_t mask;
   uint32_t starving;
-  uint32_t pad[2];
+  uint32_t hdr_waits;
+  uint32_t pad[1];
 };
 constexpr uint32_t kChunkBlocks = 2048;
 constexpr uint32_t kNoChunk = 0xFFFFFFFFu;
@@ -79,13 +83,15 @@
   aa_mb_info * mbs;
   uint32_t * chunk_list;
   uint32_t mp_stride;
-  uint32_t mp_pad;
+  uint32_t hdr_rows;
   uint32_t * packed_pos;
   unsigned long long * intra_rows;
   uint8_t * mbflags;
   FrameSummary * summary;
 };
 
+constexpr uint32_t kHdrDone = 0;
+constexpr uint32_t kHdrLeadRows = 2;
 AA_HD inline uint32_t mp_flag_index( const ParseJob & J, uint32_t row, uint32_t col )
 {
   const uint32_t P = J.fp.nparts;
@@ -270,6 +276,13 @@
   const AA_GLOBAL V16 * q = (const AA_GLOBAL V16 *) p;
   const V16 v = *q;
   Chunk16 c; c.w[0] = v.x; c.w[1] = v.y; c.w[2] = v.z; c.w[3] = v.w;
+  return c;
+}
+AA_HD inline Chunk16 load16_agent( const AA_GLOBAL uint8_t * p )
+{
+  const AA_GLOBAL uint32_t * q = (const AA_GLOBAL uint32_t *) p;
+  Chunk16 c;
+  for ( uint32_t k = 0; k < 4; k++ ) c.w[k] = AA_AT_LOAD_G( q + k );
   return c;
 }
 AA_HD inline void lds_store16( uint8_t * smem, uint32_t off, const Chunk16 & c )
@@ -318,6 +331,8 @@
   uint32_t blk_left;
   uint32_t nchunks;
   unsigned long long mem_since;
+  uint32_t hrows;
+  uint32_t hsince;
   AA_GLOBAL int16_t * sink;
   AA_GLOBAL int16_t * hdr;
   uint32_t zzmask;
@@ -392,10 +407,19 @@
   prime_stream( L, smem, J );
 }
 
+AA_HD inline const AA_GLOBAL uint32_t * hdr_rows_word( const Frame & J )
+{
+  return &J.job->hdr_rows;
+}
+AA_HD inline bool flags_written( const Frame & J, uint32_t rows, uint32_t at ) { return rows == kHdrDone || at + 16u <= ( rows - 1u ) * J.mbw; }
+constexpr uint32_t kHdrWaitTicks = 50000000u;
+
 template <bool MP = false>
 AA_HD inline void top_up( Lane & L, uint8_t * smem, const Frame & J )
 {
   if ( L.rec == R_DONE || ( MP && L.rec == R_PARK ) ) return;
+  const uint32_t rows = MP ? kHdrDone : L.hrows;
+  if constexpr ( !MP ) if ( rows != kHdrDone ) L.hrows = AA_AT_LOAD_G( hdr_rows_word( J ) );
   if ( L.pend_wpos == L.wpos ) {
     for ( uint32_t k = 0; k < kChunks; k++ )
       lds_store16( smem, L.sbase + ( ( L.wpos + 16 * k ) & ( kRing - 1 ) ), mask_past_end( L.pend[k], L.wpos + 16 * k, L.rend ) );
@@ -415,11 +439,12 @@
     }
     L.pend_wpos = L.wpos;
   }
-  if ( L.mwpos - L.mi <= kMetaRing - 16 * kMetaChunks ) {
+  static_assert( kMetaChunks == 1, "the progress word gates one chunk of flags per top-up" );
+  if ( L.mwpos - L.mi <= kMetaRing - 16 * kMetaChunks && ( MP || flags_written( J, rows, L.mwpos ) ) ) {
     for ( uint32_t k = 0; k < kMetaChunks; k++ ) {
       const uint32_t at = L.mwpos + 16 * k;
       Chunk16 c; c.w[0] = c.w[1] = c.w[2] = c.w[3] = 0;
-      if ( at < J.flags_padded ) c = load16( J.mbflags + at );
+      if ( at < J.flags_padded ) c = MP ? load16( J.mbflags + at ) : load16_agent( J.mbflags + at );
       L.mpend[k] = c;
     }
     L.pend_mwpos = L.mwpos;
@@ -619,7 +644,18 @@
   else for ( ;; ) {
     if constexpr ( MP ) if ( mp && AA_LDS_LOAD( smem, shared + offsetof( MpShared, status ) ) != TOK_OK ) { verdict = V_FINISH; break; }
     if ( L.mi == J.nmb ) { verdict = V_FINISH; break; }
-    if ( L.mi >= L.mwpos ) break;
+    if ( L.mi >= L.mwpos ) {
+      if constexpr ( !MP ) if ( !flags_written( J, L.hrows, L.mwpos ) ) {
+        const uint32_t now = static_cast<uint32_t>( AA_NOW() );
+        if ( !L.hsince ) { L.hsince = now | 1u; AA_AT_ADD( &H.pool->hdr_waits, 1u ); }
+        else if ( now - L.hsince > kHdrWaitTicks ) {
+          const uint32_t last = L.mwpos + 15u < J.nmb ? L.mwpos + 15u : J.nmb - 1u;
+          verdict = V_FINISH; status = TOK_HEADER_WAIT | ( ( last / J.mbw ) << 8 );
+        }
+      }
+      break;
+    }
+    if constexpr ( !MP ) L.hsince = 0;
     if ( L.col == J.mbw ) {
       L.col = 0; L.row++; L.ctxbits = 0;
       if constexpr ( MP ) if ( mp ) L.mi_real += ( J.mp_P - 1u ) * J.mbw;
@@ -839,7 +875,7 @@
     } while ( it < kPeriod && !AA_ANY( L.rec == R_MBDONE ) );
     if ( prof ) P.steps += it - it0;
   }
-  if ( L.rec != R_DONE ) L.steps += it;
+  if ( L.rec != R_DONE && ( MP || !L.hsince ) ) L.steps += it;
 }
 template <bool PK, bool MP = false>
 AA_HD inline void run_period( Lane & L, uint8_t * smem, const Frame & J, const Heap & H )
@@ -877,6 +913,7 @@
   L.blk = sink; L.hdr = nullptr;
   L.pend_wpos = L.pend_mwpos = kNoPend;
   L.y2byte = 0; L.nx_mi = kNoPend; L.nx_flags = L.nx_above = L.nx_y2 = 0;
+  L.hrows = kHdrDone; L.hsince = 0;
   L.steps = 0;
 }
 
@@ -909,12 +946,16 @@
     }
   }
   start_partition( L, smem, J, J.mp_P > 1 ? J.mp_p : 0u );
+  L.hrows = SH ? kHdrDone : AA_AT_LOAD_G( hdr_rows_word( J ) );
+  L.hsince = 0;
+  L.mwpos = 0;
   for ( uint32_t k = 0; k < kMetaRing / 16; k++ ) {
+    if ( !SH && !flags_written( J, L.hrows, 16 * k ) ) break;
     Chunk16 c; c.w[0] = c.w[1] = c.w[2] = c.w[3] = 0;
-    if ( 16 * k < J.flags_padded ) c = load16( J.mbflags + 16 * k );
+    if ( 16 * k < J.flags_padded ) c = SH ? load16( J.mbflags + 16 * k ) : load16_agent( J.mbflags + 16 * k );
     lds_store16( smem, base + kMeta + 16 * k, c );
-  }
-  L.mwpos = kMetaRing;
+    L.mwpos = 16 * k + 16;
+  }
   L.pend_mwpos = kNoPend;
   L.rec = R_MB;
   preload( L, smem );
diff --git a/include/alfalfa_amd.h b/include/alfalfa_amd.h
--- a/include/alfalfa_amd.h
+++ b/include/alfalfa_amd.h
@@ -246,6 +246,7 @@
   uint64_t packed_frames, packed_words, packed_blocks;
   double host_batch_ms, host_batch_parse_wall_ms, host_batch_parse_cpu_ms, host_batch_arena_ms;
   uint64_t pinned_allocs;
+  uint64_t token_header_waits;
 } aa_kernel_stats;
 aa_status aa_ctx_profile( aa_ctx * ctx, int enable );
 aa_status aa_ctx_kernel_stats( aa_ctx * ctx, aa_kernel_stats * out, int reset );
```

Result: slower. 119.9 million (-4.8%).
